# KwonGihyun/TweedieMix

Hardware: AMD Instinct MI355X
Metric: denoise steps/sec @ SDXL 1024^2 K=3 concepts (fusion phase); images/sec at 1/2/4/8 GPUs (higher is better)
Workload: dtype bf16

## Files before the change

include/tmix.h:

```cpp
#ifndef TMIX_H
#define TMIX_H

#include <stdint.h>

#ifdef __cplusplus
extern "C" {
#endif

#define TMIX_VERSION 100

enum { TMIX_OK = 0, TMIX_EINVAL = -1, TMIX_ESHAPE = -2, TMIX_EARCH = -3, TMIX_EALIGN = -4 };
enum { TMIX_F32 = 0, TMIX_F16 = 1, TMIX_BF16 = 2 };

int tmix_version(void);
const char* tmix_last_error_string(void);
int tmix_check_device(void);
void tmix_env_refresh(void);

int tmix_prof_begin(uint64_t* slots, int capacity, int detail);
int tmix_prof_end(void);

enum { TMIX_STEP_FUSION = 0, TMIX_STEP_PLAIN = 1, TMIX_STEP_RESAMPLE = 2 };
int tmix_fused_tweedie_step(const float* x, const void* eps, int eps_dtype, const float* masks,
                            float* out_x, float* out_x0, int K, int channels, int64_t hw, int mode,
// ... 10 lines not shown
int tmix_video_step_prologue(const float* x, float* x_u, int64_t clip_stride_u, float* t_u, float* x_c, int64_t clip_stride_c,
                             float* t_c, const float* params, int videos, int channels, int frames, int64_t hw, int row_channels,
                             void* stream);
int tmix_vpred_step_dev(float* x, const float* v_u, int64_t clip_stride_u, const float* v_c, int64_t clip_stride_c,
                        const float* params, int videos, int channels, int frames, int64_t hw, void* stream);
int tmix_frame_inject(void* x, int dtype, int clips, int frames, int64_t per_frame, int hard, float interp,
                      float one_minus_interp, void* stream);

enum { TMIX_EPI_NONE = 0, TMIX_EPI_GEGLU = 1, TMIX_EPI_F32OUT = 2 ,
       TMIX_EPI_GELU = 3 ,
       TMIX_EPI_QUICKGELU = 4  };
enum { TMIX_TILE_AUTO = 0, TMIX_TILE_128x128_S2 = 1, TMIX_TILE_256x128_S3 = 2, TMIX_TILE_128x128_S4 = 3,
       TMIX_TILE_256x256_S2 = 4, TMIX_TILE_256x128_W4 = 5, TMIX_TILE_256x256_W4 = 6, TMIX_TILE_128x160_S2 = 7,
       TMIX_TILE_128x160_S2_LW = 8, TMIX_TILE_256x128_S3_LW = 9, TMIX_TILE_128x128_S2_LW = 10, TMIX_TILE_256x256_S2_LW = 11,
       TMIX_TILE_128x160_S4 = 12 ,
       TMIX_TILE_64x160_W5 = 13 ,
       TMIX_TILE_256x320_S2 = 14 ,
       TMIX_TILE_32x160_W5 = 15 ,
       TMIX_TILE_256x256_PH = 16 ,
       TMIX_TILE_256x128_PH = 17,
       TMIX_TILE_128x160_S4_K2 = 18 ,
       TMIX_TILE_128x160_S3_LW = 19 ,
       TMIX_TILE_128x160_S4_LW2 = 20 ,
       TMIX_TILE_128x160_S4_LW4 = 21 ,
       TMIX_TILE_256x320_PH = 22 ,
       TMIX_TILE_128x160_W22 = 23 ,
       TMIX_TILE_CONV_HALO = 26 ,
       TMIX_TILE_COUNT = 26 };
typedef struct {
    const void* A;  int64_t lda, strideA;
    const void* W;  int64_t ldw, strideW;
    void*       C;  int64_t ldc, strideC;
    const float* bias;  int64_t strideBias;
    const void* residual; int64_t ldr, strideR;
    const float* rowgroup_bias;
    int32_t rows_per_group;
    void*   Ct; int64_t ldct, strideCt;
    int32_t n_trans_begin;
    int32_t M, N, K, batch;
    int32_t epilogue;
    int32_t tile_cfg;
    float* row_stats_out; int64_t strideStatsOut, ldStatsOut;
    const float* ln_stats; int64_t strideLnStats, ldLnStats;
    const float* ln_colsum; int64_t strideLnColsum;
    float ln_inv_c, ln_eps;
    int32_t ln_parts, reserved0;
    float* col_stats_out;
    int32_t w_period, reserved1;
} tmix_gemm_desc;
int tmix_gemm_bf16(const tmix_gemm_desc* d, void* stream);
int tmix_gemm_resolve_tile(const tmix_gemm_desc* d, int fp8_operands);
int tmix_gemm_f8copy_tile(int tile_cfg);
int tmix_gemm_prefetch_next(const void* next_weights, int64_t bytes, void* stream);
enum { TMIX_F8_A_BLOCK_SCALES = 1, TMIX_F8_GEGLU_OUT = 2, TMIX_F8_COPY_OUT = 4 };
#define TMIX_COLSTATS_ROWS 32
int tmix_gemm_fp8(const tmix_gemm_desc* d, const uint8_t* scale_a, const uint8_t* scale_w, void* stream);
int tmix_gemm_q_cross_attn(const tmix_gemm_desc* d, const void* K, int64_t ldk, int64_t strideK, const void* Vt, int64_t ldvt, int64_t strideVt,
                           void* O, int64_t ldo, int rows_per_image, int Skv, float scale, void* stream);
int tmix_quantize_fp8_rows(const void* X, int64_t ld, void* Q, int64_t ldq, uint8_t* scale_e8m0, int64_t rows, int K, void* stream);
int tmix_gemm_tile_shape(int tile_cfg, int* bm, int* bn);
int tmix_gemm_stats_parts(int N, int tile_cfg);

enum { TMIX_CONV_S1 = 0, TMIX_CONV_S2 = 1, TMIX_CONV_UP2 = 2, TMIX_CONV_T3 = 3, TMIX_CONV_S2A = 4 };
typedef struct {
    const void* X;
    const void* Wt;
    void*       Y;
    const float* bias;
    const float* batch_bias;
    const void* residual;
    int32_t B, H, W, Cin, Cout, mode;
    int32_t tile_cfg;
    int32_t batch_bias_images;
    float* col_stats_out;
    const void* S1; const void* S2;
    int32_t S1_channels, S2_channels;
} tmix_conv_desc;
int tmix_conv3x3_nhwc(const tmix_conv_desc* d, void* stream);
int tmix_conv3x3_nhwc_fp8(const tmix_conv_desc* d, const uint8_t* scale_x, const uint8_t* scale_w, void* stream);
int tmix_conv_resolve_tile(const tmix_conv_desc* d, int fp8_operands);

int tmix_conv_in(const float* x_nchw, const float* w_ohwi, const float* bias, void* y_nhwc,
                 int B, int Cin, int H, int W, int Cout, void* stream);
int tmix_conv_in_pre(const float* x_nchw, const float* w_ohwi, const float* bias, void* y_nhwc,
                     int B, int Cin, int H, int W, int Cout, const float* pre_w, const float* pre_b, void* stream);
int tmix_conv_out(const void* x_nhwc, const void* w_ohwi, const float* bias, float* y_nchw,
                  int B, int Cin, int H, int W, int Cout, void* stream);

int tmix_attn_fwd(const void* Q, int64_t ldq, int64_t strideQ, const void* K, int64_t ldk, int64_t strideK,
                  const void* Vt, int64_t ldvt, int64_t strideVt, void* O, int64_t ldo, int64_t strideO,
                  int B, int H, int Sq, int Skv, float scale, void* stream);
int tmix_attn_fwd_f8(const void* Q, int64_t ldq, int64_t strideQ, const void* K, int64_t ldk, int64_t strideK,
                     const void* Vt, int64_t ldvt, int64_t strideVt, void* O8, int64_t ldo8, void* scales, int64_t ldScale,
                     int B, int H, int Sq, int Skv, float scale, void* stream);
int64_t tmix_attn_split_ws_bytes(int B, int H, int Sq, int Skv);
int tmix_attn_fwd_ws(const void* Q, int64_t ldq, int64_t strideQ, const void* K, int64_t ldk, int64_t strideK,
                     const void* Vt, int64_t ldvt, int64_t strideVt, void* O, int64_t ldo, int64_t strideO,
                     int B, int H, int Sq, int Skv, float scale, void* ws, int64_t ws_bytes, void* stream);
int tmix_attn_fwd_f8_ws(const void* Q, int64_t ldq, int64_t strideQ, const void* K, int64_t ldk, int64_t strideK,
                        const void* Vt, int64_t ldvt, int64_t strideVt, void* O8, int64_t ldo8, void* scales, int64_t ldScale,
                        int B, int H, int Sq, int Skv, float scale, void* ws, int64_t ws_bytes, void* stream);

int64_t tmix_groupnorm_ws_floats(int B, int C, int groups);
int tmix_groupnorm_ws_chunks(int64_t HW);
int tmix_groupnorm_nhwc(const void* X1, int C1, const void* X2, int C2, void* Y, const float* gamma,
                        const float* beta, float* ws, int B, int64_t HW, int groups, float eps, int silu,
                        void* stream);
int tmix_groupnorm_nhwc_launches(int64_t HW, int C, int groups);
int tmix_groupnorm_nhwc_pre(const void* X1, int C1, const void* X2, int C2, void* Y, const float* gamma,
                            const float* beta, float* ws, int B, int64_t HW, int groups, float eps, int silu,
                            const float* cs1, int cs1_channels, const float* cs2, int cs2_channels, void* stream);
int tmix_groupnorm_nhwc_pre_f8(const void* X1, int C1, const void* X2, int C2, void* Y8, void* scales, const float* gamma,
                               const float* beta, float* ws, int B, int64_t HW, int groups, float eps, int silu,
                               const float* cs1, int cs1_channels, const float* cs2, int cs2_channels, void* stream);
int tmix_layernorm(const void* X, void* Y, const float* gamma, const float* beta, int64_t rows, int C,
                   float eps, void* stream);
int tmix_zero(void* ptr, int64_t nbytes, void* stream);
int tmix_concat_channels(const void* X1, int C1, const void* X2, int C2, void* Y, int64_t rows, void* stream);
int tmix_timestep_embedding(const float* values, float* out, int count, int dim, void* stream);
int tmix_softmax_rows(const float* S, int64_t ld_s, void* P, int64_t ld_p, int64_t rows, int cols, float scale, void* stream);
int tmix_softmax_rows_causal(const float* S, int64_t ld_s, void* P, int64_t ld_p, int64_t rows, int cols, float scale,
                             int seq, void* stream);
int tmix_softmax_rows_masked(const float* S, int64_t ld_s, void* P, int64_t ld_p, int64_t rows, int cols, int valid, float scale,
                             void* stream);
int tmix_temporal_attn(const void* QKV, int64_t ld, void* O, int64_t ldo, int clips, int frames, int64_t hw, int heads,
                       float scale, void* stream);
int tmix_lora_down(void* A, int64_t lda, int K, int64_t rows, const void* D, int P, int nsets, const float* dcolsum, const float* dbias,
                   float eps, const int* sets, int64_t rows_per_set, void* stream);
int tmix_affine_clamp(const float* x, float* y, int64_t n, float scale, float shift, float lo, float hi, void* stream);
int tmix_linear_small(const float* in, const void* W, const float* bias, const float* add, float* out,
                      int M, int N, int K, int act_in, int act_out, void* stream);
int tmix_linear_small_sections(const float* in, const void* W, const float* bias, float* out, int M, int N, int K,
                               int act_in, const int* sec_starts, int nsec, void* stream);

int tmix_conv3x3_f32(const float* x_nchw, const float* w_oihw, const float* bias, float* y_nchw, int B, int Cin, int H, int W, int Cout,
                     int stride, int silu, void* stream);
int tmix_adaptive_avgpool_f32(const float* x, float* y, int64_t planes, int H, int W, int OH, int OW, void* stream);
int tmix_linear_f32(const float* in, const float* W, const float* bias, float* out, int M, int N, int K, int act_in, int act_out, void* stream);
int tmix_i2v_temporal_encoder(const float* x, float* y, int clips, int frames, int channels, int64_t hw, const float* ln_gamma, const float* ln_beta,
                              const float* wq, const float* wk, const float* wv, const float* wo, const float* bo,
                              const float* w1, const float* b1, const float* w2, const float* b2, void* stream);

int tmix_xattn_token_maps(const void* Q, int64_t ldq, int64_t strideQ, const void* K, int64_t ldk, int64_t strideK, float* maps,
                          int B, int H, int Sq, int Lk, int row0, int row_step, int n_rows, const int32_t* tokens, int n_tok,
                          int accumulate, float scale, void* stream);

#ifdef __cplusplus
}
#endif
#endif
```

tweediemix_amd/csrc/norm_misc.hip:

```cpp
#include "common.h"

namespace {

typedef __attribute__((ext_vector_type(8))) __bf16 frag_ab;

__device__ __forceinline__ void unpack8(const uint4& v, float (&f)[8]) {
    f[0] = bf2f((bf16_t)(v.x & 0xffff)); f[1] = bf2f((bf16_t)(v.x >> 16));
    f[2] = bf2f((bf16_t)(v.y & 0xffff)); f[3] = bf2f((bf16_t)(v.y >> 16));
    f[4] = bf2f((bf16_t)(v.z & 0xffff)); f[5] = bf2f((bf16_t)(v.z >> 16));
    f[6] = bf2f((bf16_t)(v.w & 0xffff)); f[7] = bf2f((bf16_t)(v.w >> 16));
}
__device__ __forceinline__ uint4 pack8(const float (&f)[8]) {
    uint4 v;
    v.x = pack_bf2(f[0], f[1]); v.y = pack_bf2(f[2], f[3]); v.z = pack_bf2(f[4], f[5]); v.w = pack_bf2(f[6], f[7]);
    return v;
}

constexpr int GN_MAX_C = 4096;

#ifndef GN_T
#define GN_T 128
#endif
#ifndef GN_APPLY_U
#define GN_APPLY_U 2
// ... 61 lines not shown
        float* o = ws + (((int64_t)b * chunks + ch) * groups + tid) * 2;
        o[0] = s; o[1] = q;
    }
}

__global__ void __launch_bounds__(64) gn_finalize_kernel(const float* __restrict__ ws, const float* __restrict__ gamma,
                                                         const float* __restrict__ beta, float2* __restrict__ ss,
                                                         int C, int64_t HW, int groups, int chunks, float eps) {
    const int g = blockIdx.x, b = blockIdx.y, lane = threadIdx.x, cpg = C / groups;
    double s = 0.0, q = 0.0;
    for (int ch = lane; ch < chunks; ch += 64) {
        const float* o = ws + (((int64_t)b * chunks + ch) * groups + g) * 2;
        s += (double)o[0]; q += (double)o[1];
    }
#pragma unroll
    for (int o = 32; o > 0; o >>= 1) { s += __shfl_xor(s, o); q += __shfl_xor(q, o); }
    const double n = (double)HW * cpg;
    const double mean = s / n;
    double var = q / n - mean * mean; if (var < 0.0) var = 0.0;
    const float meanf = (float)mean, rstd = (float)(1.0 / sqrt(var + (double)eps));
    for (int c = g * cpg + lane; c < (g + 1) * cpg; c += 64) {
        const float sc = rstd * gamma[c];
        ss[(int64_t)b * C + c] = make_float2(sc, beta[c] - meanf * sc);
    }
}

constexpr int GN_CS_T = 1024;
__device__ __forceinline__ void gn_cs_walk(const float* __restrict__ base, int Cs, int n, int nblk, int tid, float& s, float& q) {
    if (n <= 0) return;
    const int J = GN_CS_T / n, j = tid / n, c = tid - j * n;
    if (j >= J) return;
    const float* row = base + (int64_t)j * 2 * Cs + c;
    const int64_t step = (int64_t)J * 2 * Cs;
    int blk = j;
    for (; blk + 3 * J < nblk; blk += 4 * J, row += 4 * step) {
        const float a0 = row[0], b0 = row[Cs], a1 = row[step], b1 = row[step + Cs];
        const float a2 = row[2 * step], b2 = row[2 * step + Cs], a3 = row[3 * step], b3 = row[3 * step + Cs];
        s += (a0 + a1) + (a2 + a3); q += (b0 + b1) + (b2 + b3);
    }
    for (; blk < nblk; blk += J, row += step) { s += row[0]; q += row[Cs]; }
}
__global__ void __launch_bounds__(GN_CS_T) gn_finalize_cs_kernel(const float* __restrict__ cs1, int C1, const float* __restrict__ cs2, int C2,
                                                                 const float* __restrict__ gamma, const float* __restrict__ beta,
                                                                 float2* __restrict__ ss, int64_t HW, int groups, float eps,
                                                                 unsigned long long* prof) {
    __shared__ double s_red[2 * GN_CS_T / 64];
    __shared__ float s_ms[2];
    if (prof && threadIdx.x == 0) prof_enter(prof, (blockIdx.x | blockIdx.y) == 0, 0);
    const int C = C1 + C2, cpg = C / groups;
    const int g = blockIdx.x, b = blockIdx.y, tid = threadIdx.x;
    const int nblk = (int)(HW / 32);
    float gm = 0.f, bt = 0.f;
    if (tid < cpg) { gm = gamma[g * cpg + tid]; bt = beta[g * cpg + tid]; }
    const int c_lo = g * cpg, c_hi = c_lo + cpg;
    const int n1 = min(c_hi, C1) - min(c_lo, C1), n2 = cpg - n1;
    float s = 0.f, q = 0.f;
    gn_cs_walk(cs1 + (int64_t)b * nblk * 2 * C1 + c_lo, C1, n1, nblk, tid, s, q);
    if (n2 > 0) gn_cs_walk(cs2 + (int64_t)b * nblk * 2 * C2 + (max(c_lo, C1) - C1), C2, n2, nblk, tid, s, q);
    double sd = (double)s, qd = (double)q;
#pragma unroll
    for (int o = 32; o > 0; o >>= 1) { sd += __shfl_xor(sd, o); qd += __shfl_xor(qd, o); }
    if ((tid & 63) == 0) { s_red[(tid >> 6) * 2] = sd; s_red[(tid >> 6) * 2 + 1] = qd; }
    __syncthreads();
    if (tid == 0) {
        double st = 0.0, qt = 0.0;
#pragma unroll
        for (int w = 0; w < GN_CS_T / 64; ++w) { st += s_red[2 * w]; qt += s_red[2 * w + 1]; }
        const double n = (double)HW * cpg;
        const double mean = st / n;
        double var = qt / n - mean * mean; if (var < 0.0) var = 0.0;
        s_ms[0] = (float)mean; s_ms[1] = (float)(1.0 / sqrt(var + (double)eps));
    }
    __syncthreads();
    if (tid < cpg) {
        const float sc = s_ms[1] * gm;
        ss[(int64_t)b * C + c_lo + tid] = make_float2(sc, bt - s_ms[0] * sc);
    }
}

__device__ __forceinline__ float silu_fast(float x) {
    return x * __builtin_amdgcn_rcpf(1.0f + __builtin_amdgcn_exp2f(-1.4426950408889634f * x));
}

__device__ __forceinline__ float gn_quad_max(float x) {
    float y = __int_as_float(__builtin_amdgcn_update_dpp(0, __float_as_int(x), 0xB1, 0xf, 0xf, false));
    x = fmaxf(x, y);
    y = __int_as_float(__builtin_amdgcn_update_dpp(0, __float_as_int(x), 0x4E, 0xf, 0xf, false));
    return fmaxf(x, y);
}

template <int F8>
__global__ void __launch_bounds__(256) gn_apply_kernel(const bf16_t* __restrict__ X1, int C1, const bf16_t* __restrict__ X2, int C2,
                                                       bf16_t* __restrict__ Y, const float2* __restrict__ ss, int64_t HW, int silu,
                                                       unsigned long long* prof, unsigned char* __restrict__ Y8 = nullptr, unsigned char* __restrict__ S8 = nullptr) {
    __shared__ float2 s_ss[GN_MAX_C];
    const unsigned long long pt0 = (prof && threadIdx.x == 0) ? prof_now() : 0;
    const int C = C1 + C2, nvec = C >> 3;
    const int b = blockIdx.y, tid = threadIdx.x;
    for (int c = tid; c < C; c += 256) s_ss[c] = ss[(int64_t)b * C + c];
    __syncthreads();
    const int64_t total = HW * nvec;
    int64_t per = (total + gridDim.x - 1) / gridDim.x;
    if (F8) per = (per + 3) & ~(int64_t)3;
    const int64_t i0 = (int64_t)blockIdx.x * per;
    int64_t i1 = i0 + per; if (i1 > total) i1 = total;
    int64_t p = i0 / nvec; int v = (int)(i0 - p * nvec) + tid;
    while (v >= nvec) { v -= nvec; ++p; }
    const int step_p = 256 / nvec, step_v = 256 - step_p * nvec;
    constexpr int U = GN_APPLY_U;
    for (int64_t i = i0 + tid; i < i1; i += 256 * U) {
        uint4 raw[U]; int64_t pp[U]; int cc[U];
#pragma unroll
        for (int u = 0; u < U; ++u) {
            pp[u] = p; cc[u] = v * 8;
            if (i + u * 256 < i1) {
                const bf16_t* src = (cc[u] < C1) ? X1 + ((int64_t)b * HW + p) * C1 + cc[u] : X2 + ((int64_t)b * HW + p) * C2 + (cc[u] - C1);
                raw[u] = *(const uint4*)src;
            }
            p += step_p; v += step_v;
            if (v >= nvec) { v -= nvec; ++p; }
        }
#pragma unroll
        for (int u = 0; u < U; ++u) {
            if (i + u * 256 < i1) {
                float f[8]; unpack8(raw[u], f);
#pragma unroll
                for (int j = 0; j < 8; ++j) {
                    const float2 k = s_ss[cc[u] + j];
                    float y = f[j] * k.x + k.y;
                    if (silu) y = silu_fast(y);
                    f[j] = y;
                }
                if constexpr (F8) {
                    const uint4 pk = pack8(f);
                    unpack8(pk, f);
                    float am = 0.f;
#pragma unroll
                    for (int j = 0; j < 8; ++j) am = fmaxf(am, fabsf(f[j]));
                    am = gn_quad_max(am);
                    const int e = e8m0_for_amax(am);
                    const float inv = exp2_neg_int(e);
                    int q0 = __builtin_amdgcn_cvt_pk_fp8_f32(f[0] * inv, f[1] * inv, 0, false); q0 = __builtin_amdgcn_cvt_pk_fp8_f32(f[2] * inv, f[3] * inv, q0, true);
                    int q1 = __builtin_amdgcn_cvt_pk_fp8_f32(f[4] * inv, f[5] * inv, 0, false); q1 = __builtin_amdgcn_cvt_pk_fp8_f32(f[6] * inv, f[7] * inv, q1, true);
                    const int64_t row = (int64_t)b * HW + pp[u];
                    *(uint2*)(Y8 + row * C + cc[u]) = make_uint2((unsigned)q0, (unsigned)q1);
                    if ((tid & 3) == 0) S8[row * (C >> 5) + (cc[u] >> 5)] = (unsigned char)(e + 127);
                } else
                *(uint4*)(Y + ((int64_t)b * HW + pp[u]) * C + cc[u]) = pack8(f);
            }
        }
    }
    if (prof && threadIdx.x == 0) prof_leave(prof, 0, pt0, pt0, pt0);
}

constexpr int GN_SMALL_MAX_CW = 256, GN_SMALL_MAX_ELEMS = 65536;
__global__ void __launch_bounds__(256) gn_small_kernel(const bf16_t* __restrict__ X1, int C1, const bf16_t* __restrict__ X2, int C2, bf16_t* __restrict__ Y,
                                                       const float* __restrict__ gamma, const float* __restrict__ beta, int HW, int groups, int gpw, float eps, int silu,
                                                       unsigned long long* prof) {
    __shared__ float r_s[2048], r_q[2048];
    __shared__ double c_s[GN_SMALL_MAX_CW], c_q[GN_SMALL_MAX_CW];
    __shared__ float g_ms[16];
    __shared__ float2 s_ss[GN_SMALL_MAX_CW];
    const unsigned long long pt0 = (prof && threadIdx.x == 0) ? prof_enter(prof, (blockIdx.x | blockIdx.y) == 0, 0) : 0;
    const int C = C1 + C2, cpg = C / groups, cw = gpw * cpg, nv = cw >> 3, rs = 256 / nv;
    const int b = blockIdx.y, c0 = blockIdx.x * cw, tid = threadIdx.x;
    const int v = tid % nv, slot = tid / nv;
    const bool active = slot < rs;
    const int cg = c0 + v * 8;
    const bf16_t* src; int ld;
    if (cg < C1) { src = X1 + (int64_t)b * HW * C1 + cg; ld = C1; } else { src = X2 + (int64_t)b * HW * C2 + (cg - C1); ld = C2; }
    float s[8], q[8];
#pragma unroll
    for (int j = 0; j < 8; ++j) { s[j] = 0.f; q[j] = 0.f; }
    if (active) {
        int row = slot;
        for (; row + 3 * rs < HW; row += 4 * rs) {
            uint4 raw[4];
#pragma unroll
            for (int u = 0; u < 4; ++u) raw[u] = *(const uint4*)(src + (int64_t)(row + u * rs) * ld);
#pragma unroll
            for (int u = 0; u < 4; ++u) {
                float f[8]; unpack8(raw[u], f);
#pragma unroll
                for (int j = 0; j < 8; ++j) { s[j] += f[j]; q[j] += f[j] * f[j]; }
            }
        }
        for (; row < HW; row += rs) {
            float f[8]; unpack8(*(const uint4*)(src + (int64_t)row * ld), f);
#pragma unroll
            for (int j = 0; j < 8; ++j) { s[j] += f[j]; q[j] += f[j] * f[j]; }
        }
#pragma unroll
        for (int j = 0; j < 8; ++j) { r_s[slot * cw + v * 8 + j] = s[j]; r_q[slot * cw + v * 8 + j] = q[j]; }
    }
    __syncthreads();
    if (tid < cw) {
        double a = 0.0, d = 0.0;
        for (int k = 0; k < rs; ++k) { a += (double)r_s[k * cw + tid]; d += (double)r_q[k * cw + tid]; }
        c_s[tid] = a; c_q[tid] = d;
    }
    __syncthreads();
    if (tid < gpw) {
        double a = 0.0, d = 0.0;
        for (int k = 0; k < cpg; ++k) { a += c_s[tid * cpg + k]; d += c_q[tid * cpg + k]; }
        const double n = (double)HW * cpg, mean = a / n;
        double var = d / n - mean * mean; if (var < 0.0) var = 0.0;
        g_ms[2 * tid] = (float)mean; g_ms[2 * tid + 1] = (float)(1.0 / sqrt(var + (double)eps));
    }
    __syncthreads();
    if (tid < cw) {
        const int g = tid / cpg;
        const float sc = g_ms[2 * g + 1] * gamma[c0 + tid];
        s_ss[tid] = make_float2(sc, beta[c0 + tid] - g_ms[2 * g] * sc);
    }
    __syncthreads();
    if (active) {
        float2 k[8];
#pragma unroll
        for (int j = 0; j < 8; ++j) k[j] = s_ss[v * 8 + j];
        bf16_t* dst = Y + (int64_t)b * HW * C + cg;
        int row = slot;
        for (; row + 3 * rs < HW; row += 4 * rs) {
            uint4 raw[4];
#pragma unroll
            for (int u = 0; u < 4; ++u) raw[u] = *(const uint4*)(src + (int64_t)(row + u * rs) * ld);
#pragma unroll
            for (int u = 0; u < 4; ++u) {
                float f[8]; unpack8(raw[u], f);
#pragma unroll
                for (int j = 0; j < 8; ++j) { float y = f[j] * k[j].x + k[j].y; if (silu) y = silu_fast(y); f[j] = y; }
                *(uint4*)(dst + (int64_t)(row + u * rs) * C) = pack8(f);
            }
        }
        for (; row < HW; row += rs) {
            float f[8]; unpack8(*(const uint4*)(src + (int64_t)row * ld), f);
#pragma unroll
            for (int j = 0; j < 8; ++j) { float y = f[j] * k[j].x + k[j].y; if (silu) y = silu_fast(y); f[j] = y; }
            *(uint4*)(dst + (int64_t)row * C) = pack8(f);
        }
    }
    if (prof && threadIdx.x == 0) prof_leave(prof, 0, pt0, pt0, pt0);
}
static int gn_small_gpw(int64_t HW, int C, int groups) {
    if (tmix_env(TMIX_ENV_GN_NO_SMALL)) return 0;
    const int cpg = C / groups;
    for (int gpw = 1; gpw <= 8; gpw <<= 1) {
        if (groups % gpw || ((gpw * cpg) & 7)) continue;
        const int cw = gpw * cpg;
        if (cw > GN_SMALL_MAX_CW || HW * cw > GN_SMALL_MAX_ELEMS) return 0;
        return gpw;
    }
    return 0;
}

__global__ void __launch_bounds__(256) layernorm_kernel(const bf16_t* __restrict__ X, bf16_t* __restrict__ Y,
                                                        const float* __restrict__ gamma, const float* __restrict__ beta,
                                                        int64_t rows, int C, float eps) {
    const int lane = threadIdx.x & 63;
    const int64_t row = (int64_t)blockIdx.x * 4 + (threadIdx.x >> 6);
    if (row >= rows) return;
    const int nvec = C >> 3;
    float f[4][8];
    float s = 0.f;
#pragma unroll
    for (int i = 0; i < 4; ++i) {
        const int v = i * 64 + lane;
        if (v < nvec) {
            const uint4 raw = *(const uint4*)(X + row * C + v * 8);
            unpack8(raw, f[i]);
#pragma unroll
            for (int j = 0; j < 8; ++j) s += f[i][j];
        }
    }
#pragma unroll
    for (int o = 32; o > 0; o >>= 1) s += __shfl_xor(s, o);
    const float mean = s / (float)C;
    float q = 0.f;
#pragma unroll
    for (int i = 0; i < 4; ++i) {
        const int v = i * 64 + lane;
        if (v < nvec) {
#pragma unroll
            for (int j = 0; j < 8; ++j) { const float d = f[i][j] - mean; q += d * d; }
        }
    }
#pragma unroll
    for (int o = 32; o > 0; o >>= 1) q += __shfl_xor(q, o);
    const float rstd = rsqrtf(q / (float)C + eps);
#pragma unroll
    for (int i = 0; i < 4; ++i) {
        const int v = i * 64 + lane;
        if (v < nvec) {
            const float4 g0 = *(const float4*)(gamma + v * 8), g1 = *(const float4*)(gamma + v * 8 + 4);
            const float4 b0 = *(const float4*)(beta + v * 8), b1 = *(const float4*)(beta + v * 8 + 4);
            const float gg[8] = {g0.x, g0.y, g0.z, g0.w, g1.x, g1.y, g1.z, g1.w};
            const float bb[8] = {b0.x, b0.y, b0.z, b0.w, b1.x, b1.y, b1.z, b1.w};
            float y[8];
#pragma unroll
            for (int j = 0; j < 8; ++j) y[j] = (f[i][j] - mean) * rstd * gg[j] + bb[j];
            *(uint4*)(Y + row * C + v * 8) = pack8(y);
        }
    }
}

__global__ void __launch_bounds__(256) softmax_rows_kernel(const float* __restrict__ S, int64_t ld_s, bf16_t* __restrict__ P,
                                                           int64_t ld_p, int cols, float scale_log2e, int seq, int valid) {
    __shared__ float red[4];
    const float* row = S + (int64_t)blockIdx.x * ld_s;
    bf16_t* out = P + (int64_t)blockIdx.x * ld_p;
    const int tid = threadIdx.x, lane = tid & 63, w = tid >> 6;
    const int lim = seq > 0 ? (int)(blockIdx.x % (unsigned)seq) + 1 : valid;
    auto load = [&](int c) {
        float4 v = *(const float4*)(row + c);
        if (c + 0 >= lim) v.x = -INFINITY;
        if (c + 1 >= lim) v.y = -INFINITY;
        if (c + 2 >= lim) v.z = -INFINITY;
        if (c + 3 >= lim) v.w = -INFINITY;
        return v;
    };
    float mx = -INFINITY;
    for (int c = tid * 4; c < cols; c += 1024) {
        const float4 v = load(c);
        mx = fmaxf(fmaxf(mx, fmaxf(v.x, v.y)), fmaxf(v.z, v.w));
    }
#pragma unroll
    for (int o = 32; o > 0; o >>= 1) mx = fmaxf(mx, __shfl_xor(mx, o));
    if (lane == 0) red[w] = mx;
    __syncthreads();
    mx = fmaxf(fmaxf(red[0], red[1]), fmaxf(red[2], red[3])) * scale_log2e;
    __syncthreads();
    float sum = 0.f;
    for (int c = tid * 4; c < cols; c += 1024) {
        const float4 v = load(c);
        sum += exp2f(v.x * scale_log2e - mx) + exp2f(v.y * scale_log2e - mx) + exp2f(v.z * scale_log2e - mx) + exp2f(v.w * scale_log2e - mx);
    }
// ... 63 lines not shown
                float xf[8] = {x0.x, x0.y, x0.z, x0.w, x1.x, x1.y, x1.z, x1.w};
                if (act_in) {
#pragma unroll
                    for (int j = 0; j < 8; ++j) xf[j] = silu_f(xf[j]);
                }
#pragma unroll
                for (int j = 0; j < 8; ++j) acc[m] += xf[j] * wf[j];
            }
        }
    }
#pragma unroll
    for (int m = 0; m < MAXM; ++m) {
#pragma unroll
        for (int o = 32; o > 0; o >>= 1) acc[m] += __shfl_xor(acc[m], o);
    }
    if (lane == 0) {
        int64_t base = 0; int ldn = N, col = n;
        if (secs) {
            int sidx = 0;
            while (sidx + 1 < nsec && secs[sidx + 1] <= n) ++sidx;
            base = (int64_t)secs[sidx] * Mtot; ldn = secs[sidx + 1] - secs[sidx]; col = n - secs[sidx];
        }
        for (int m = 0; m < M; ++m) {
            float y = acc[m] + (bias ? bias[n] : 0.f) + (add ? add[(int64_t)m * N + n] : 0.f);
            if (act_out) y = silu_f(y);
            out[base + (int64_t)(secs ? mrow0 + m : m) * ldn + col] = y;
        }
    }
}

struct PreMap { float w[16]; float b[4]; int on; };

template <int CIN>
__global__ void __launch_bounds__(256) conv_in_kernel(const float* __restrict__ x, const float* __restrict__ w,
                                                      const float* __restrict__ bias, bf16_t* __restrict__ y,
                                                      int B, int H, int W, int Cout, const PreMap pm) {
    extern __shared__ __attribute__((aligned(16))) float s_w[];
    constexpr int KK = 9 * CIN;
    const int tid = threadIdx.x, lane = tid & 63;
    const int q = __builtin_amdgcn_readfirstlane(tid >> 6);
    for (int i = tid; i < Cout * KK / 4; i += 256) ((float4*)s_w)[i] = ((const float4*)w)[i];
    __syncthreads();
    const int64_t npix = (int64_t)B * H * W;
    for (int64_t tile = blockIdx.x; tile * 64 < npix; tile += gridDim.x) {
    int64_t pix = tile * 64 + lane;
    const bool live = pix < npix;
    if (!live) pix = npix - 1;
    const int b = (int)(pix / ((int64_t)H * W)); const int rem = (int)(pix - (int64_t)b * H * W);
    const int oy = rem / W, ox = rem - oy * W;
    float patch[KK];
#pragma unroll
    for (int ky = 0; ky < 3; ++ky)
#pragma unroll
        for (int kx = 0; kx < 3; ++kx) {
            const int iy = oy + ky - 1, ix = ox + kx - 1;
            const bool ok = iy >= 0 && iy < H && ix >= 0 && ix < W;
            float v[CIN];
#pragma unroll
            for (int ci = 0; ci < CIN; ++ci) v[ci] = ok ? x[(((int64_t)b * CIN + ci) * H + iy) * W + ix] : 0.f;
            if (pm.on && CIN == 4) {
                float u[4];
#pragma unroll
                for (int co = 0; co < 4; ++co)
                    u[co] = ok ? pm.b[co] + pm.w[co * 4 + 0] * v[0] + pm.w[co * 4 + 1] * v[1] + pm.w[co * 4 + 2] * v[2] + pm.w[co * 4 + 3] * v[3] : 0.f;
#pragma unroll
                for (int co = 0; co < 4; ++co) v[co] = u[co];
            }
#pragma unroll
            for (int ci = 0; ci < CIN; ++ci) patch[(ky * 3 + kx) * CIN + ci] = v[ci];
        }
    const int cpq = Cout / 4;
    for (int c0 = q * cpq; c0 < (q + 1) * cpq; c0 += 8) {
        float o[8];
#pragma unroll 2
        for (int j = 0; j < 8; ++j) {
            const float* wr = s_w + (c0 + j) * KK;
            float a = bias ? bias[c0 + j] : 0.f;
#pragma unroll
            for (int k = 0; k < KK; ++k) a += patch[k] * wr[k];
            o[j] = a;
        }
        if (live) *(uint4*)(y + pix * Cout + c0) = pack8(o);
    }
    }
}

__global__ void __launch_bounds__(256) conv_out_kernel(const bf16_t* __restrict__ x, const bf16_t* __restrict__ w,
                                                       const float* __restrict__ bias, float* __restrict__ y,
                                                       int B, int H, int W, int Cin, int Cout) {
    const int lane = threadIdx.x & 63, fr = lane & 15, fg = lane >> 4;
    const int64_t npix = (int64_t)B * H * W;
    const int64_t pbase = ((int64_t)blockIdx.x * 4 + (threadIdx.x >> 6)) * 16;
    if (pbase >= npix) return;
    int64_t pix = pbase + fr; if (pix > npix - 1) pix = npix - 1;
    const int b = (int)(pix / ((int64_t)H * W)); const int rem = (int)(pix - (int64_t)b * H * W);
    const int oy = rem / W, ox = rem - oy * W;
    const int co = fr < Cout ? fr : Cout - 1;
    const bf16_t* wrow = w + (int64_t)co * 9 * Cin;
    f32x4 acc = {0.f, 0.f, 0.f, 0.f};
    const frag_ab zero = {0, 0, 0, 0, 0, 0, 0, 0};
    for (int tap = 0; tap < 9; ++tap) {
        const int ky = tap / 3, kx = tap - ky * 3;
        const int iy = oy + ky - 1, ix = ox + kx - 1;
        const bool ok = iy >= 0 && iy < H && ix >= 0 && ix < W;
        const bf16_t* src = x + (((int64_t)b * H + (ok ? iy : 0)) * W + (ok ? ix : 0)) * Cin;
        for (int c = 0; c < Cin; c += 32) {
            frag_ab a = *(const frag_ab*)(src + c + fg * 8);
            if (!ok) a = zero;
            const frag_ab wf = *(const frag_ab*)(wrow + tap * Cin + c + fg * 8);
            acc = __builtin_amdgcn_mfma_f32_16x16x32_bf16(a, wf, acc, 0, 0, 0);
        }
    }
    if (fr < Cout) {
        const float bv = bias ? bias[fr] : 0.f;
#pragma unroll
        for (int r = 0; r < 4; ++r) {
            const int64_t pp = pbase + fg * 4 + r;
            if (pp < npix) {
                const int bb = (int)(pp / ((int64_t)H * W)); const int64_t rr = pp - (int64_t)bb * H * W;
                y[((int64_t)bb * Cout + fr) * H * W + rr] = acc[r] + bv;
            }
        }
    }
}

}

extern "C" int tmix_groupnorm_ws_chunks(int64_t HW) { return gn_chunks(HW); }
extern "C" int64_t tmix_groupnorm_ws_floats(int B, int C, int groups) { return (int64_t)B * GN_T * groups * 2 + (int64_t)B * C * 2; }

extern "C" int tmix_groupnorm_nhwc_launches(int64_t HW, int C, int groups) {
    if (HW <= 0 || C <= 0 || groups <= 0 || (C % groups)) return 0;
    return gn_small_gpw(HW, C, groups) ? 1 : 3;
}

extern "C" int tmix_groupnorm_nhwc(const void* X1, int C1, const void* X2, int C2, void* Y, const float* gamma,
                                   const float* beta, float* ws, int B, int64_t HW, int groups, float eps, int silu,
                                   void* stream) {
    if (!X1 || !Y || !gamma || !beta || !ws) TMIX_FAIL(TMIX_EINVAL, "groupnorm: null pointer");
    if (C2 > 0 && !X2) TMIX_FAIL(TMIX_EINVAL, "groupnorm: C2 > 0 but X2 is null");
    const int C = C1 + C2;
    if (B <= 0 || HW <= 0 || C <= 0) TMIX_FAIL(TMIX_ESHAPE, "groupnorm: empty problem");
    if ((C1 % 8) || (C2 % 8) || C > GN_MAX_C || groups <= 0 || groups > 64 || (C % groups)) TMIX_FAIL(TMIX_ESHAPE, "groupnorm: C1=%d C2=%d groups=%d unsupported", C1, C2, groups);
    if (!aligned16(X1) || (X2 && !aligned16(X2)) || !aligned16(Y)) TMIX_FAIL(TMIX_EALIGN, "groupnorm: pointers must be 16-byte aligned");
    const int chunks = gn_chunks(HW);
    hipStream_t st = (hipStream_t)stream;
    unsigned long long* prof = tmix_prof_take();
    if (const int gpw = gn_small_gpw(HW, C, groups)) {
        gn_small_kernel<<<dim3(groups / gpw, B), 256, 0, st>>>((const bf16_t*)X1, C1, (const bf16_t*)X2, C2, (bf16_t*)Y, gamma, beta, (int)HW, groups, gpw, eps, silu, prof);
        TMIX_LAUNCH_CHECK();
        return TMIX_OK;
    }
    gn_stats_kernel<<<dim3(chunks, B), 256, 0, st>>>((const bf16_t*)X1, C1, (const bf16_t*)X2, C2, ws, HW, groups, chunks, prof);
    TMIX_LAUNCH_CHECK();
    float2* ss = (float2*)(ws + (int64_t)B * GN_T * groups * 2);
    gn_finalize_kernel<<<dim3(groups, B), 64, 0, st>>>(ws, gamma, beta, ss, C, HW, groups, chunks, eps);
    TMIX_LAUNCH_CHECK();
    int64_t nb = (HW * (C / 8) + GN_APPLY_ITEMS - 1) / GN_APPLY_ITEMS; if (nb < 1) nb = 1; if (nb > GN_APPLY_MAXB) nb = GN_APPLY_MAXB;
    gn_apply_kernel<0><<<dim3((unsigned)nb, B), 256, 0, st>>>((const bf16_t*)X1, C1, (const bf16_t*)X2, C2, (bf16_t*)Y, ss, HW, silu, prof);
    TMIX_LAUNCH_CHECK();
    return TMIX_OK;
}

static int gn_pre_entry(const void* X1, int C1, const void* X2, int C2, void* Y, void* S8, const float* gamma,
                        const float* beta, float* ws, int B, int64_t HW, int groups, float eps, int silu,
                        const float* cs1, int cs1_channels, const float* cs2, int cs2_channels, void* stream) {
    if (!X1 || !Y || !gamma || !beta || !ws || !cs1) TMIX_FAIL(TMIX_EINVAL, "groupnorm_pre: null pointer");
    if (S8 && ((C1 + C2) % 32)) TMIX_FAIL(TMIX_ESHAPE, "groupnorm_pre_f8: C must be a multiple of 32 (MX blocks)");
    if (C2 > 0 && !X2) TMIX_FAIL(TMIX_EINVAL, "groupnorm_pre: C2 > 0 but X2 is null");
    const int C = C1 + C2;
    if (cs1_channels <= 0 || cs2_channels < 0 || cs1_channels + cs2_channels != C || (cs2_channels > 0 && !cs2))
        TMIX_FAIL(TMIX_EINVAL, "groupnorm_pre: the partials cover %d + %d channels, the tensor has %d", cs1_channels, cs2_channels, C);
    if (B <= 0 || HW <= 0 || C <= 0) TMIX_FAIL(TMIX_ESHAPE, "groupnorm_pre: empty problem");
    if ((C1 % 8) || (C2 % 8) || C > GN_MAX_C || groups <= 0 || groups > 64 || (C % groups) || C / groups > 256) TMIX_FAIL(TMIX_ESHAPE, "groupnorm_pre: C1=%d C2=%d groups=%d unsupported", C1, C2, groups);
    if (HW % TMIX_COLSTATS_ROWS) TMIX_FAIL(TMIX_ESHAPE, "groupnorm_pre: HW=%lld must be a multiple of %d (the producers' partials cover 32-row blocks)", (long long)HW, TMIX_COLSTATS_ROWS);
    if (!aligned16(X1) || (X2 && !aligned16(X2)) || !aligned16(Y)) TMIX_FAIL(TMIX_EALIGN, "groupnorm_pre: pointers must be 16-byte aligned");
    hipStream_t st = (hipStream_t)stream;
    unsigned long long* prof = tmix_prof_take();
    float2* ss = (float2*)(ws + (int64_t)B * GN_T * groups * 2);
    gn_finalize_cs_kernel<<<dim3(groups, B), GN_CS_T, 0, st>>>(cs1, cs1_channels, cs2, cs2_channels, gamma, beta, ss, HW, groups, eps, prof);
    TMIX_LAUNCH_CHECK();
    int64_t nb = (HW * (C / 8) + GN_APPLY_ITEMS - 1) / GN_APPLY_ITEMS; if (nb < 1) nb = 1; if (nb > GN_APPLY_MAXB) nb = GN_APPLY_MAXB;
    if (S8) gn_apply_kernel<1><<<dim3((unsigned)nb, B), 256, 0, st>>>((const bf16_t*)X1, C1, (const bf16_t*)X2, C2, nullptr, ss, HW, silu, prof, (unsigned char*)Y, (unsigned char*)S8);
    else gn_apply_kernel<0><<<dim3((unsigned)nb, B), 256, 0, st>>>((const bf16_t*)X1, C1, (const bf16_t*)X2, C2, (bf16_t*)Y, ss, HW, silu, prof);
    TMIX_LAUNCH_CHECK();
    return TMIX_OK;
}

extern "C" int tmix_groupnorm_nhwc_pre(const void* X1, int C1, const void* X2, int C2, void* Y, const float* gamma,
                                       const float* beta, float* ws, int B, int64_t HW, int groups, float eps, int silu,
                                       const float* cs1, int cs1_channels, const float* cs2, int cs2_channels, void* stream) {
    return gn_pre_entry(X1, C1, X2, C2, Y, nullptr, gamma, beta, ws, B, HW, groups, eps, silu, cs1, cs1_channels, cs2, cs2_channels, stream);
}

extern "C" int tmix_groupnorm_nhwc_pre_f8(const void* X1, int C1, const void* X2, int C2, void* Y8, void* scales, const float* gamma,
                                          const float* beta, float* ws, int B, int64_t HW, int groups, float eps, int silu,
                                          const float* cs1, int cs1_channels, const float* cs2, int cs2_channels, void* stream) {
    if (!scales) TMIX_FAIL(TMIX_EINVAL, "groupnorm_pre_f8: null scale array");
    return gn_pre_entry(X1, C1, X2, C2, Y8, scales, gamma, beta, ws, B, HW, groups, eps, silu, cs1, cs1_channels, cs2, cs2_channels, stream);
}

extern "C" int tmix_layernorm(const void* X, void* Y, const float* gamma, const float* beta, int64_t rows, int C,
                              float eps, void* stream) {
    if (!X || !Y || !gamma || !beta) TMIX_FAIL(TMIX_EINVAL, "layernorm: null pointer");
    if (rows <= 0 || C <= 0) TMIX_FAIL(TMIX_ESHAPE, "layernorm: empty problem");
    if ((C % 8) || C > 2048) TMIX_FAIL(TMIX_ESHAPE, "layernorm: C=%d must be a multiple of 8 and <= 2048", C);
    if (!aligned16(X) || !aligned16(Y) || !aligned16(gamma) || !aligned16(beta)) TMIX_FAIL(TMIX_EALIGN, "layernorm: pointers must be 16-byte aligned");
    layernorm_kernel<<<(unsigned)((rows + 3) / 4), 256, 0, (hipStream_t)stream>>>((const bf16_t*)X, (bf16_t*)Y, gamma, beta, rows, C, eps);
    TMIX_LAUNCH_CHECK();
    return TMIX_OK;
}

__global__ void __launch_bounds__(256) quantize_fp8_rows_kernel(const bf16_t* __restrict__ X, int64_t ld, unsigned char* __restrict__ Q, int64_t ldq,
                                                                unsigned char* __restrict__ scale, int64_t rows, int K) {
    const int lane = threadIdx.x & 63;
    const int64_t r = (int64_t)blockIdx.x * 4 + (threadIdx.x >> 6);
    if (r >= rows) return;
    constexpr int MAXV = 16;
    const int nv = K >> 3;
    uint4 v[MAXV];
    float amax = 0.f;
#pragma unroll
    for (int u = 0; u < MAXV; ++u) {
        const int c = u * 64 + lane;
        if (c < nv) {
            v[u] = *(const uint4*)(X + r * ld + (int64_t)c * 8);
            const unsigned w[4] = {v[u].x, v[u].y, v[u].z, v[u].w};
#pragma unroll
            for (int k = 0; k < 4; ++k) amax = fmaxf(amax, fmaxf(fabsf(__uint_as_float(w[k] << 16)), fabsf(__uint_as_float(w[k] & 0xffff0000u))));
        }
    }
#pragma unroll
    for (int off = 32; off >= 1; off >>= 1) amax = fmaxf(amax, __shfl_xor(amax, off));
    const int e = e8m0_for_amax(amax);
    const float inv = exp2_neg_int(e);
    if (lane == 0) scale[r] = (unsigned char)(e + 127);
#pragma unroll
    for (int u = 0; u < MAXV; ++u) {
        const int c = u * 64 + lane;
        if (c < nv) {
            const unsigned w[4] = {v[u].x, v[u].y, v[u].z, v[u].w};
            unsigned o[2];
#pragma unroll
            for (int h = 0; h < 2; ++h) {
                const float f0 = __uint_as_float(w[2 * h] << 16) * inv, f1 = __uint_as_float(w[2 * h] & 0xffff0000u) * inv;
                const float f2 = __uint_as_float(w[2 * h + 1] << 16) * inv, f3 = __uint_as_float(w[2 * h + 1] & 0xffff0000u) * inv;
                int pk = __builtin_amdgcn_cvt_pk_fp8_f32(f0, f1, 0, false);
                pk = __builtin_amdgcn_cvt_pk_fp8_f32(f2, f3, pk, true);
                o[h] = (unsigned)pk;
            }
            *(uint2*)(Q + r * ldq + (int64_t)c * 8) = make_uint2(o[0], o[1]);
        }
    }
}

extern "C" int tmix_quantize_fp8_rows(const void* X, int64_t ld, void* Q, int64_t ldq, uint8_t* scale_e8m0, int64_t rows, int K, void* stream) {
    if (!X || !Q || !scale_e8m0) TMIX_FAIL(TMIX_EINVAL, "quantize_fp8_rows: null pointer");
    if (rows <= 0 || K <= 0 || (K % 8) || K > 8192) TMIX_FAIL(TMIX_ESHAPE, "quantize_fp8_rows: rows=%lld K=%d (K %% 8 == 0, K <= 8192)", (long long)rows, K);
    if (!aligned16(X) || (ld % 8) || (((uintptr_t)Q) & 7) || (ldq % 8)) TMIX_FAIL(TMIX_EALIGN, "quantize_fp8_rows: X rows must be 16-byte, Q rows 8-byte aligned");
    quantize_fp8_rows_kernel<<<(unsigned)((rows + 3) / 4), 256, 0, (hipStream_t)stream>>>((const bf16_t*)X, ld, (unsigned char*)Q, ldq, scale_e8m0, rows, K);
    TMIX_LAUNCH_CHECK();
    return TMIX_OK;
}

extern "C" int tmix_zero(void* ptr, int64_t nbytes, void* stream) {
    if (!ptr || nbytes <= 0) TMIX_FAIL(TMIX_EINVAL, "zero: null pointer / empty range");
    hipError_t e = hipMemsetAsync(ptr, 0, (size_t)nbytes, (hipStream_t)stream);
    if (e != hipSuccess) TMIX_FAIL((int)e, "hipMemsetAsync: %s", hipGetErrorString(e));
    return TMIX_OK;
}

extern "C" int tmix_concat_channels(const void* X1, int C1, const void* X2, int C2, void* Y, int64_t rows, void* stream) {
    if (!X1 || !X2 || !Y) TMIX_FAIL(TMIX_EINVAL, "concat: null pointer");
    if (rows <= 0 || C1 <= 0 || C2 <= 0 || (C1 % 8) || (C2 % 8)) TMIX_FAIL(TMIX_ESHAPE, "concat: rows=%lld C1=%d C2=%d unsupported", (long long)rows, C1, C2);
    if (!aligned16(X1) || !aligned16(X2) || !aligned16(Y)) TMIX_FAIL(TMIX_EALIGN, "concat: pointers must be 16-byte aligned");
    int64_t nb = (rows * ((C1 + C2) / 8) + 255) / 256; if (nb > 4096) nb = 4096;
    concat_kernel<<<(unsigned)nb, 256, 0, (hipStream_t)stream>>>((const uint4*)X1, C1 / 8, (const uint4*)X2, C2 / 8, (uint4*)Y, rows);
    TMIX_LAUNCH_CHECK();
    return TMIX_OK;
}

namespace {
// ... 200 lines not shown
extern "C" int tmix_timestep_embedding(const float* values, float* out, int count, int dim, void* stream) {
    if (!values || !out) TMIX_FAIL(TMIX_EINVAL, "timestep_embedding: null pointer");
    if (count <= 0 || dim <= 0 || (dim & 1)) TMIX_FAIL(TMIX_ESHAPE, "timestep_embedding: count=%d dim=%d", count, dim);
    const int n = count * (dim / 2);
    timestep_embedding_kernel<<<(n + 255) / 256, 256, 0, (hipStream_t)stream>>>(values, out, count, dim);
    TMIX_LAUNCH_CHECK();
    return TMIX_OK;
}

static int linear_small_launch(const float* in, const void* W, const float* bias, const float* add, float* out, int M, int N, int K,
                               int act_in, int act_out, const int* secs, int nsec, hipStream_t st) {
    for (int m0 = 0; m0 < M; m0 += 16) {
        const int m = M - m0 < 16 ? M - m0 : 16;
        const float* in_c = in + (int64_t)m0 * K;
        const float* add_c = add ? add + (int64_t)m0 * N : nullptr;
        float* out_c = secs ? out : out + (int64_t)m0 * N;
        if (m <= 4) linear_small_kernel<4><<<(N + 3) / 4, 256, 0, st>>>(in_c, (const bf16_t*)W, bias, add_c, out_c, m, N, K, act_in, act_out, secs, nsec, M, m0);
        else        linear_small_kernel<16><<<(N + 3) / 4, 256, 0, st>>>(in_c, (const bf16_t*)W, bias, add_c, out_c, m, N, K, act_in, act_out, secs, nsec, M, m0);
        TMIX_LAUNCH_CHECK();
    }
    return TMIX_OK;
}

extern "C" int tmix_linear_small(const float* in, const void* W, const float* bias, const float* add, float* out,
                                 int M, int N, int K, int act_in, int act_out, void* stream) {
    if (!in || !W || !out) TMIX_FAIL(TMIX_EINVAL, "linear_small: null pointer");
    if (M <= 0 || M > 256 || N <= 0 || K <= 0 || (K % 8)) TMIX_FAIL(TMIX_ESHAPE, "linear_small: M=%d (1..256) N=%d K=%d (K %% 8 == 0)", M, N, K);
    if (!aligned16(in) || !aligned16(W)) TMIX_FAIL(TMIX_EALIGN, "linear_small: in/W must be 16-byte aligned");
    return linear_small_launch(in, W, bias, add, out, M, N, K, act_in, act_out, nullptr, 0, (hipStream_t)stream);
}

extern "C" int tmix_linear_small_sections(const float* in, const void* W, const float* bias, float* out, int M, int N, int K,
                                          int act_in, const int* sec_starts, int nsec, void* stream) {
    if (!in || !W || !out || !sec_starts) TMIX_FAIL(TMIX_EINVAL, "linear_small_sections: null pointer");
    if (M <= 0 || M > 256 || N <= 0 || K <= 0 || (K % 8) || nsec < 1) TMIX_FAIL(TMIX_ESHAPE, "linear_small_sections: M=%d (1..256) N=%d K=%d (K %% 8 == 0) nsec=%d", M, N, K, nsec);
    if (!aligned16(in) || !aligned16(W)) TMIX_FAIL(TMIX_EALIGN, "linear_small_sections: in/W must be 16-byte aligned");
    return linear_small_launch(in, W, bias, nullptr, out, M, N, K, act_in, 0, sec_starts, nsec, (hipStream_t)stream);
}

extern "C" int tmix_conv_in(const float* x_nchw, const float* w_ohwi, const float* bias, void* y_nhwc,
                            int B, int Cin, int H, int W, int Cout, void* stream) {
    return tmix_conv_in_pre(x_nchw, w_ohwi, bias, y_nhwc, B, Cin, H, W, Cout, nullptr, nullptr, stream);
}

extern "C" int tmix_conv_in_pre(const float* x_nchw, const float* w_ohwi, const float* bias, void* y_nhwc,
                                int B, int Cin, int H, int W, int Cout, const float* pre_w, const float* pre_b, void* stream) {
    if (!x_nchw || !w_ohwi || !y_nhwc) TMIX_FAIL(TMIX_EINVAL, "conv_in: null pointer");
    if (B <= 0 || H <= 0 || W <= 0 || Cout <= 0) TMIX_FAIL(TMIX_ESHAPE, "conv_in: bad shape");
    if (!aligned16(y_nhwc)) TMIX_FAIL(TMIX_EALIGN, "conv_in: output must be 16-byte aligned");
    if (Cout % 32) TMIX_FAIL(TMIX_ESHAPE, "conv_in: Cout=%d must be a multiple of 32", Cout);
    if (Cin != 3 && Cin != 4 && Cin != 8) TMIX_FAIL(TMIX_ESHAPE, "conv_in: Cin=%d (3: RGB image, 4: image latent, 8: video latent + image-latent features)", Cin);
    if (Cin != 4 && pre_w) TMIX_FAIL(TMIX_EINVAL, "conv_in: the latent pre-map is defined for 4 channels");
    if ((Cout * 9 * Cin) % 4) TMIX_FAIL(TMIX_ESHAPE, "conv_in: Cout*9*Cin must be a multiple of 4");
    if (!aligned16(w_ohwi)) TMIX_FAIL(TMIX_EALIGN, "conv_in: weights must be 16-byte aligned");
    const int64_t npix = (int64_t)B * H * W;
    const int64_t ntiles = (npix + 63) / 64;
    const int smem = Cout * 9 * Cin * 4;
    const int per_cu = smem > 80 * 1024 ? 1 : (smem > 52 * 1024 ? 2 : 3);
    const unsigned nb = (unsigned)(ntiles < 256 * per_cu ? ntiles : 256 * per_cu);
    if (smem > 150 * 1024) TMIX_FAIL(TMIX_ESHAPE, "conv_in: Cout=%d too large for the LDS weight stage", Cout);
    static int attr_smem[3] = {0, 0, 0};
    const int slot = Cin == 8 ? 2 : (Cin == 4 ? 1 : 0);
    if (smem > 64 * 1024 && smem > attr_smem[slot]) {
        hipError_t e = Cin == 8 ? hipFuncSetAttribute((const void*)conv_in_kernel<8>, hipFuncAttributeMaxDynamicSharedMemorySize, smem)
                     : Cin == 4 ? hipFuncSetAttribute((const void*)conv_in_kernel<4>, hipFuncAttributeMaxDynamicSharedMemorySize, smem)
                                : hipFuncSetAttribute((const void*)conv_in_kernel<3>, hipFuncAttributeMaxDynamicSharedMemorySize, smem);
        if (e != hipSuccess) TMIX_FAIL((int)e, "hipFuncSetAttribute: %s", hipGetErrorString(e));
        attr_smem[slot] = smem;
    }
    PreMap pm = {};
    if (pre_w) {
        pm.on = 1;
        for (int i = 0; i < 16; ++i) pm.w[i] = pre_w[i];
        for (int i = 0; i < 4; ++i) pm.b[i] = pre_b ? pre_b[i] : 0.f;
    }
    hipStream_t st = (hipStream_t)stream;
    if (Cin == 8) conv_in_kernel<8><<<nb, 256, smem, st>>>(x_nchw, w_ohwi, bias, (bf16_t*)y_nhwc, B, H, W, Cout, pm);
    else if (Cin == 3) conv_in_kernel<3><<<nb, 256, smem, st>>>(x_nchw, w_ohwi, bias, (bf16_t*)y_nhwc, B, H, W, Cout, pm);
    else          conv_in_kernel<4><<<nb, 256, smem, st>>>(x_nchw, w_ohwi, bias, (bf16_t*)y_nhwc, B, H, W, Cout, pm);
    TMIX_LAUNCH_CHECK();
    return TMIX_OK;
}

extern "C" int tmix_conv_out(const void* x_nhwc, const void* w_ohwi, const float* bias, float* y_nchw,
                             int B, int Cin, int H, int W, int Cout, void* stream) {
    if (!x_nhwc || !w_ohwi || !y_nchw) TMIX_FAIL(TMIX_EINVAL, "conv_out: null pointer");
    if (B <= 0 || H <= 0 || W <= 0 || Cout <= 0 || Cout > 16 || (Cin % 32)) TMIX_FAIL(TMIX_ESHAPE, "conv_out: Cin=%d (%%32) Cout=%d (<=16)", Cin, Cout);
    if (!aligned16(x_nhwc) || !aligned16(w_ohwi)) TMIX_FAIL(TMIX_EALIGN, "conv_out: pointers must be 16-byte aligned");
    const int64_t npix = (int64_t)B * H * W;
    const unsigned nb = (unsigned)((npix + 63) / 64);
    conv_out_kernel<<<nb, 256, 0, (hipStream_t)stream>>>((const bf16_t*)x_nhwc, (const bf16_t*)w_ohwi, bias, y_nchw, B, H, W, Cin, Cout);
    TMIX_LAUNCH_CHECK();
    return TMIX_OK;
}
```

tweediemix_amd/lib.py:

```python
from __future__ import annotations

import ctypes as C
import os

_HERE = os.path.dirname(os.path.abspath(__file__))
LIB_PATH = os.path.join(_HERE, "lib", "libtmix_hip.so")
LIB_PATH = os.environ.get("TMIX_LIB", LIB_PATH)

OK, EINVAL, ESHAPE, EARCH, EALIGN = 0, -1, -2, -3, -4
F32, F16, BF16 = 0, 1, 2
STEP_FUSION, STEP_PLAIN, STEP_RESAMPLE = 0, 1, 2
EPI_NONE, EPI_GEGLU, EPI_F32OUT, EPI_GELU, EPI_QUICKGELU = 0, 1, 2, 3, 4
CONV_S1, CONV_S2, CONV_UP2, CONV_T3, CONV_S2A = 0, 1, 2, 3, 4
F8_A_BLOCK_SCALES, F8_GEGLU_OUT, F8_COPY_OUT = 1, 2, 4
TILE_AUTO, TILE_COUNT = 0, 26
TILE_CANDIDATES = (1, 2, 3, 4, 5, 7, 12, 13, 14, 15, 16, 17, 18, 19, 20, 21, 22)
TILE_EXCLUSIVE = (13, 14, 15, 22, 24)
TILE_CONV_HALO = 26

i32, i64, f32, vp = C.c_int32, C.c_int64, C.c_float, C.c_void_p


class GemmDesc(C.Structure):
    _fields_ = [("A", vp), ("lda", i64), ("strideA", i64),
                ("W", vp), ("ldw", i64), ("strideW", i64),
                ("C", vp), ("ldc", i64), ("strideC", i64),
                ("bias", vp), ("strideBias", i64),
                ("residual", vp), ("ldr", i64), ("strideR", i64),
                ("rowgroup_bias", vp), ("rows_per_group", i32),
                ("Ct", vp), ("ldct", i64), ("strideCt", i64),
                ("n_trans_begin", i32),
                ("M", i32), ("N", i32), ("K", i32), ("batch", i32),
                ("epilogue", i32), ("tile_cfg", i32),
                ("row_stats_out", vp), ("strideStatsOut", i64), ("ldStatsOut", i64),
                ("ln_stats", vp), ("strideLnStats", i64), ("ldLnStats", i64),
                ("ln_colsum", vp), ("strideLnColsum", i64), ("ln_inv_c", f32), ("ln_eps", f32),
                ("ln_parts", C.c_int32), ("reserved0", C.c_int32),
                ("col_stats_out", vp), ("w_period", C.c_int32), ("reserved1", C.c_int32)]


class ConvDesc(C.Structure):
    _fields_ = [("X", vp), ("Wt", vp), ("Y", vp), ("bias", vp), ("batch_bias", vp), ("residual", vp),
                ("B", i32), ("H", i32), ("W", i32), ("Cin", i32), ("Cout", i32), ("mode", i32), ("tile_cfg", i32),
                ("batch_bias_images", i32), ("col_stats_out", vp), ("S1", vp), ("S2", vp), ("S1_channels", i32), ("S2_channels", i32)]


SIGNATURES = {
    "tmix_version": (C.c_int, []),
    "tmix_last_error_string": (C.c_char_p, []),
    "tmix_check_device": (C.c_int, []),
    "tmix_env_refresh": (None, []),
    "tmix_prof_begin": (C.c_int, [vp, C.c_int, C.c_int]),
    "tmix_prof_end": (C.c_int, []),
    "tmix_fused_tweedie_step": (C.c_int, [vp, vp, C.c_int, vp, vp, vp, C.c_int, C.c_int, i64, C.c_int,
                                          f32, f32, f32, f32, f32, C.c_int, vp]),
    "tmix_fused_tweedie_step_dev": (C.c_int, [vp, vp, C.c_int, vp, i64, vp, vp, C.c_int, C.c_int, i64, C.c_int, C.c_int,
                                              C.c_int, vp, vp]),
    "tmix_step_prologue": (C.c_int, [vp, vp, vp, vp, C.c_int, C.c_int, i64, vp]),
    "tmix_gemm_bf16": (C.c_int, [C.POINTER(GemmDesc), vp]),
    "tmix_gemm_prefetch_next": (C.c_int, [vp, i64, vp]),
    "tmix_gemm_fp8": (C.c_int, [C.POINTER(GemmDesc), vp, vp, vp]),
    "tmix_gemm_q_cross_attn": (C.c_int, [C.POINTER(GemmDesc), vp, i64, i64, vp, i64, i64, vp, i64, C.c_int, C.c_int, f32, vp]),
    "tmix_quantize_fp8_rows": (C.c_int, [vp, i64, vp, i64, vp, i64, C.c_int, vp]),
    "tmix_conv3x3_nhwc": (C.c_int, [C.POINTER(ConvDesc), vp]),
    "tmix_conv3x3_nhwc_fp8": (C.c_int, [C.POINTER(ConvDesc), vp, vp, vp]),
    "tmix_conv_in": (C.c_int, [vp, vp, vp, vp, C.c_int, C.c_int, C.c_int, C.c_int, C.c_int, vp]),
    "tmix_conv_in_pre": (C.c_int, [vp, vp, vp, vp, C.c_int, C.c_int, C.c_int, C.c_int, C.c_int, vp, vp, vp]),
    "tmix_softmax_rows": (C.c_int, [vp, i64, vp, i64, i64, C.c_int, f32, vp]),
    "tmix_softmax_rows_causal": (C.c_int, [vp, i64, vp, i64, i64, C.c_int, f32, C.c_int, vp]),
    "tmix_softmax_rows_masked": (C.c_int, [vp, i64, vp, i64, i64, C.c_int, C.c_int, f32, vp]),
    "tmix_affine_clamp": (C.c_int, [vp, vp, i64, f32, f32, f32, f32, vp]),
    "tmix_conv_out": (C.c_int, [vp, vp, vp, vp, C.c_int, C.c_int, C.c_int, C.c_int, C.c_int, vp]),
    "tmix_attn_fwd": (C.c_int, [vp, i64, i64, vp, i64, i64, vp, i64, i64, vp, i64, i64,
                                C.c_int, C.c_int, C.c_int, C.c_int, f32, vp]),
    "tmix_attn_fwd_f8": (C.c_int, [vp, i64, i64, vp, i64, i64, vp, i64, i64, vp, i64, vp, i64,
                                   C.c_int, C.c_int, C.c_int, C.c_int, f32, vp]),
    "tmix_attn_split_ws_bytes": (i64, [C.c_int, C.c_int, C.c_int, C.c_int]),
    "tmix_attn_fwd_ws": (C.c_int, [vp, i64, i64, vp, i64, i64, vp, i64, i64, vp, i64, i64,
                                   C.c_int, C.c_int, C.c_int, C.c_int, f32, vp, i64, vp]),
    "tmix_attn_fwd_f8_ws": (C.c_int, [vp, i64, i64, vp, i64, i64, vp, i64, i64, vp, i64, vp, i64,
                                      C.c_int, C.c_int, C.c_int, C.c_int, f32, vp, i64, vp]),
    "tmix_groupnorm_nhwc_launches": (C.c_int, [i64, C.c_int, C.c_int]),
    "tmix_groupnorm_ws_chunks": (C.c_int, [i64]),
    "tmix_groupnorm_ws_floats": (i64, [C.c_int, C.c_int, C.c_int]),
    "tmix_groupnorm_nhwc": (C.c_int, [vp, C.c_int, vp, C.c_int, vp, vp, vp, vp, C.c_int, i64, C.c_int, f32,
                                      C.c_int, vp]),
    "tmix_groupnorm_nhwc_pre": (C.c_int, [vp, C.c_int, vp, C.c_int, vp, vp, vp, vp, C.c_int, i64, C.c_int, f32,
                                          C.c_int, vp, C.c_int, vp, C.c_int, vp]),
    "tmix_groupnorm_nhwc_pre_f8": (C.c_int, [vp, C.c_int, vp, C.c_int, vp, vp, vp, vp, vp, C.c_int, i64, C.c_int, f32,
                                             C.c_int, vp, C.c_int, vp, C.c_int, vp]),
    "tmix_layernorm": (C.c_int, [vp, vp, vp, vp, i64, C.c_int, f32, vp]),
    "tmix_zero": (C.c_int, [vp, i64, vp]),
    "tmix_temporal_attn": (C.c_int, [vp, i64, vp, i64, C.c_int, C.c_int, i64, C.c_int, f32, vp]),
    "tmix_vpred_step": (C.c_int, [vp, vp, vp, C.c_int, i64, f32, f32, f32, f32, f32, vp]),
    "tmix_frame_inject": (C.c_int, [vp, C.c_int, C.c_int, C.c_int, i64, C.c_int, f32, f32, vp]),
    "tmix_video_step_prologue": (C.c_int, [vp, vp, i64, vp, vp, i64, vp, vp, C.c_int, C.c_int, C.c_int, i64, C.c_int, vp]),
    "tmix_vpred_step_dev": (C.c_int, [vp, vp, i64, vp, i64, vp, C.c_int, C.c_int, C.c_int, i64, vp]),
    "tmix_gemm_tile_shape": (C.c_int, [C.c_int, C.POINTER(C.c_int), C.POINTER(C.c_int)]),
    "tmix_gemm_stats_parts": (C.c_int, [C.c_int, C.c_int]),
    "tmix_gemm_resolve_tile": (C.c_int, [C.POINTER(GemmDesc), C.c_int]),
    "tmix_conv_resolve_tile": (C.c_int, [C.POINTER(ConvDesc), C.c_int]),
    "tmix_gemm_f8copy_tile": (C.c_int, [C.c_int]),
    "tmix_concat_channels": (C.c_int, [vp, C.c_int, vp, C.c_int, vp, i64, vp]),
    "tmix_lora_down": (C.c_int, [vp, i64, C.c_int, i64, vp, C.c_int, C.c_int, vp, vp, f32, vp, i64, vp]),
    "tmix_timestep_embedding": (C.c_int, [vp, vp, C.c_int, C.c_int, vp]),
    "tmix_linear_small": (C.c_int, [vp, vp, vp, vp, vp, C.c_int, C.c_int, C.c_int, C.c_int, C.c_int, vp]),
    "tmix_linear_small_sections": (C.c_int, [vp, vp, vp, vp, C.c_int, C.c_int, C.c_int, C.c_int, vp, C.c_int, vp]),
    "tmix_conv3x3_f32": (C.c_int, [vp, vp, vp, vp] + [C.c_int] * 7 + [vp]),
    "tmix_adaptive_avgpool_f32": (C.c_int, [vp, vp, C.c_int64, C.c_int, C.c_int, C.c_int, C.c_int, vp]),
    "tmix_linear_f32": (C.c_int, [vp, vp, vp, vp, C.c_int, C.c_int, C.c_int, C.c_int, C.c_int, vp]),
    "tmix_i2v_temporal_encoder": (C.c_int, [vp, vp, C.c_int, C.c_int, C.c_int, C.c_int64] + [vp] * 11 + [vp]),
    "tmix_xattn_token_maps": (C.c_int, [vp, i64, i64, vp, i64, i64, vp, C.c_int, C.c_int, C.c_int, C.c_int, C.c_int, C.c_int, C.c_int,
                                        C.POINTER(C.c_int32), C.c_int, C.c_int, f32, vp]),
}

_lib = None


class TmixError(RuntimeError):
    pass


def load() -> C.CDLL:
    global _lib
    if _lib is not None:
        return _lib
    import torch
    if not os.path.exists(LIB_PATH):
        raise ImportError(f"{LIB_PATH} not found: build it first (python -c 'import __graft_entry__ as g; g.build()' "
                          f"or make -C tweediemix_amd/csrc). There is no CPU fallback.")
    lib = C.CDLL(LIB_PATH)
    for name, (res, args) in SIGNATURES.items():
        fn = getattr(lib, name)
        fn.restype = res
        fn.argtypes = args
    if lib.tmix_version() != 100:
        raise ImportError(f"libtmix_hip.so ABI version {lib.tmix_version()} != 100")
    _lib = lib
    return lib


def check(rc: int, what: str = "") -> None:
    if rc != 0:
        msg = load().tmix_last_error_string().decode("utf-8", "replace")
        raise TmixError(f"{what} failed with code {rc}: {msg}")
```

tweediemix_amd/ops.py:

```python
from __future__ import annotations

import ctypes as C

import numpy as np
import torch

from . import lib as L

BF16 = torch.bfloat16


def _stream() -> int:
    return torch.cuda.current_stream().cuda_stream


def _p(t):
    return None if t is None else t.data_ptr()


def _need_cuda(*ts):
    for t in ts:
        if t is not None and not t.is_cuda:
            raise L.TmixError("tweediemix_amd ops need device tensors (no CPU fallback exists)")

# ... 232 lines not shown
    if f8_copy is not None:
        f8_copy.attach(d)
    L.check(lib.tmix_gemm_fp8(C.byref(d), sa.data_ptr(), sw.data_ptr(), _stream()), "tmix_gemm_fp8")
    return out if out is not None else kw.get("out_f32")


def make_conv_desc(x, w, out, bias=None, batch_bias=None, residual=None, mode=L.CONV_S1, tile_cfg=0, bias_images=1, col_stats_out=None,
                   shortcut=None, _fp8=False):
    B, H, W, Cin = x.shape
    Cout = w.shape[0]
    dt = torch.uint8 if _fp8 else BF16
    assert x.dtype == dt and w.dtype == dt and x.is_contiguous() and w.is_contiguous() and out.is_contiguous()
    if shortcut is not None:
        s1, s2 = shortcut
        c1, c2 = s1.shape[-1], (0 if s2 is None else s2.shape[-1])
        assert mode == L.CONV_S1 and tuple(w.shape) == (Cout, 9 * Cin + c1 + c2) and residual is None
        assert s1.dtype == BF16 and s1.is_contiguous() and s1.numel() == B * H * W * c1 and (s2 is None or (s2.dtype == BF16 and s2.is_contiguous() and s2.numel() == B * H * W * c2))
    else:
        assert tuple(w.shape) == ((Cout, 3, Cin) if mode == L.CONV_T3 else (Cout, 3, 3, Cin))
    d = L.ConvDesc()
    d.X, d.Wt, d.Y = x.data_ptr(), w.data_ptr(), out.data_ptr()
    d.bias, d.batch_bias, d.residual = _p(bias), _p(batch_bias), _p(residual)
    d.B, d.H, d.W, d.Cin, d.Cout, d.mode = B, H, W, Cin, Cout, mode
    d.tile_cfg = tile_cfg
    d.batch_bias_images = bias_images
    if col_stats_out is not None:
        cs = col_stats_out
        assert cs.dtype == torch.float32 and cs.is_contiguous() and tuple(cs.shape) == (out.numel() // Cout // COLSTATS_ROWS, 2, Cout)
        d.col_stats_out = cs.data_ptr()
    if shortcut is not None:
        d.S1, d.S1_channels = s1.data_ptr(), c1
        if s2 is not None:
            d.S2, d.S2_channels = s2.data_ptr(), c2
    return d


def shortcut_weight(w_conv, w_sc):
    Cout = w_conv.shape[0]
    return torch.cat([w_conv.reshape(Cout, -1), w_sc.reshape(Cout, -1)], dim=1).contiguous()


def conv_out_hw(H, W, mode):
    return (H // 2, W // 2) if mode in (L.CONV_S2, L.CONV_S2A) else ((2 * H, 2 * W) if mode == L.CONV_UP2 else (H, W))


def conv3x3_fp8(x8, sx, w8, sw, bias=None, batch_bias=None, residual=None, mode=L.CONV_S1, out=None, tile_cfg=12, col_stats_out=None, bias_images=1):
    _need_cuda(x8, w8, sx, sw)
    lib = L.load()
    B, H, W, Cin = x8.shape
    Ho, Wo = conv_out_hw(H, W, mode)
    if out is None:
        out = torch.empty(B, Ho, Wo, w8.shape[0], device=x8.device, dtype=BF16)
    assert x8.dtype == torch.uint8 and w8.dtype == torch.uint8 and sx.dtype == torch.uint8 and sw.dtype == torch.uint8
    assert x8.is_contiguous() and w8.is_contiguous() and sx.is_contiguous() and sw.is_contiguous() and sx.numel() == B * H * W * Cin // 32 and sw.numel() == w8.shape[0]
    d = make_conv_desc(x8, w8, out, bias, batch_bias, residual, mode, tile_cfg, bias_images=bias_images, col_stats_out=col_stats_out, _fp8=True)
    L.check(lib.tmix_conv3x3_nhwc_fp8(C.byref(d), sx.data_ptr(), sw.data_ptr(), _stream()), "tmix_conv3x3_nhwc_fp8")
    return out


def conv3x3(x, w, bias=None, batch_bias=None, residual=None, mode=L.CONV_S1, out=None, tile_cfg=0, col_stats_out=None, shortcut=None):
    _need_cuda(x, w)
    lib = L.load()
    B, H, W, _ = x.shape
    Ho, Wo = conv_out_hw(H, W, mode)
    if out is None:
        out = torch.empty(B, Ho, Wo, w.shape[0], device=x.device, dtype=BF16)
    d = make_conv_desc(x, w, out, bias, batch_bias, residual, mode, tile_cfg, col_stats_out=col_stats_out, shortcut=shortcut)
    L.check(lib.tmix_conv3x3_nhwc(C.byref(d), _stream()), "tmix_conv3x3_nhwc")
    return out


def conv_in(x_nchw, w_ohwi, bias, out=None):
    _need_cuda(x_nchw, w_ohwi)
    lib = L.load()
    B, Cin, H, W = x_nchw.shape
    Cout = w_ohwi.shape[0]
    assert x_nchw.dtype == torch.float32 and w_ohwi.dtype == torch.float32 and x_nchw.is_contiguous() and w_ohwi.is_contiguous()
    if out is None:
        out = torch.empty(B, H, W, Cout, device=x_nchw.device, dtype=BF16)
    L.check(lib.tmix_conv_in(_p(x_nchw), _p(w_ohwi), _p(bias), _p(out), B, Cin, H, W, Cout, _stream()), "tmix_conv_in")
    return out


def conv_out(x_nhwc, w_ohwi, bias, out=None):
    _need_cuda(x_nhwc, w_ohwi)
    lib = L.load()
    B, H, W, Cin = x_nhwc.shape
    Cout = w_ohwi.shape[0]
    assert x_nhwc.dtype == BF16 and w_ohwi.dtype == BF16 and x_nhwc.is_contiguous() and w_ohwi.is_contiguous()
    if out is None:
        out = torch.empty(B, Cout, H, W, device=x_nhwc.device, dtype=torch.float32)
    L.check(lib.tmix_conv_out(_p(x_nhwc), _p(w_ohwi), _p(bias), _p(out), B, Cin, H, W, Cout, _stream()), "tmix_conv_out")
    return out


def attention_split_ws(B, H, Sq, Skv, device):
    n = L.load().tmix_attn_split_ws_bytes(B, H, Sq, Skv)
    return torch.zeros(n, device=device, dtype=torch.uint8) if n > 0 else None


def attention(q, k, vt, H, Skv, scale, out=None, f8_out=None, ws=None):
    _need_cuda(q, k, vt)
    lib = L.load()
    B, Sq = q.shape[0], q.shape[1]
    assert q.dtype == BF16 and k.dtype == BF16 and vt.dtype == BF16
    assert q.stride(2) == 1 and k.stride(2) == 1 and vt.stride(2) == 1
    wsa = (ws.data_ptr(), ws.numel()) if ws is not None else (None, 0)
    if f8_out is not None:
        assert f8_out.rows == B * Sq and f8_out.N == H * 64
        L.check(lib.tmix_attn_fwd_f8_ws(_p(q), q.stride(1), q.stride(0), _p(k), k.stride(1), k.stride(0), _p(vt), vt.stride(1), vt.stride(0),
                                        f8_out.q.data_ptr(), f8_out.N, f8_out.scales.data_ptr(), f8_out.rows,
                                        B, H, Sq, Skv, float(scale), *wsa, _stream()), "tmix_attn_fwd_f8_ws")
        return f8_out
    if out is None:
        out = torch.empty(B, Sq, H * 64, device=q.device, dtype=BF16)
    L.check(lib.tmix_attn_fwd_ws(_p(q), q.stride(1), q.stride(0), _p(k), k.stride(1), k.stride(0),
                                 _p(vt), vt.stride(1), vt.stride(0), _p(out), out.stride(1), out.stride(0),
                                 B, H, Sq, Skv, float(scale), *wsa, _stream()), "tmix_attn_fwd_ws")
    return out


def token_array(tokens):
    tokens = [int(t) for t in tokens]
    return (C.c_int32 * max(1, len(tokens)))(*tokens)


def xattn_token_maps(q, k, tokens, H, Lk=None, rows=(0, 1, None), scale=None, out=None, accumulate=False):
    _need_cuda(q, k)
    assert q.dtype == BF16 and k.dtype == BF16 and q.stride(2) == 1 and k.stride(2) == 1
    B, Sq = q.shape[0], q.shape[1]
    Lk = k.shape[1] if Lk is None else Lk
    row0, step, n = rows
    n = len(range(row0, B, step)) if n is None else n
    if out is None:
        out = torch.zeros(n, len(tokens), Sq, device=q.device, dtype=torch.float32)
    assert out.dtype == torch.float32 and out.is_contiguous() and tuple(out.shape) == (n, len(tokens), Sq)
    scale = 64 ** -0.5 if scale is None else scale
    L.check(L.load().tmix_xattn_token_maps(_p(q), q.stride(1), q.stride(0), _p(k), k.stride(1), k.stride(0), _p(out), B, H, Sq, Lk,
                                           row0, step, n, token_array(tokens), len(tokens), int(bool(accumulate)), float(scale),
                                           _stream()), "tmix_xattn_token_maps")
    return out


def groupnorm_ws(B, C, groups, device):
    return torch.empty(L.load().tmix_groupnorm_ws_floats(B, C, groups), device=device, dtype=torch.float32)


def groupnorm(x1, gamma, beta, groups=32, eps=1e-5, silu=False, x2=None, out=None, ws=None, colstats=None, f8_out=None):
    _need_cuda(x1, gamma, beta)
    lib = L.load()
    B, HW, C1 = x1.shape[0], x1.numel() // (x1.shape[0] * x1.shape[-1]), x1.shape[-1]
    C2 = 0 if x2 is None else x2.shape[-1]
    assert x1.is_contiguous() and (x2 is None or x2.is_contiguous()) and gamma.dtype == torch.float32
    assert f8_out is None or colstats is not None, "the e4m3 output exists for the producer-statistics form (tmix_groupnorm_nhwc_pre_f8)"
    if out is None and f8_out is None:
        out = torch.empty(*x1.shape[:-1], C1 + C2, device=x1.device, dtype=BF16)
    if ws is None:
        ws = groupnorm_ws(B, C1 + C2, groups, x1.device)
    if colstats is not None:
        cs1, cs2 = colstats
        ca, cb = cs1.shape[-1], (0 if cs2 is None else cs2.shape[-1])
        assert cs1.is_contiguous() and cs1.shape[1] == 2 and (cs2 is None or (cs2.is_contiguous() and cs2.shape[:2] == cs1.shape[:2]))
        if HW % COLSTATS_ROWS == 0:
            assert cs1.shape[0] == B * HW // COLSTATS_ROWS
        if f8_out is not None:
            y8, s8 = f8_out
            assert y8.dtype == torch.uint8 and s8.dtype == torch.uint8 and y8.is_contiguous() and s8.is_contiguous()
            assert y8.numel() == B * HW * (C1 + C2) and s8.numel() == B * HW * (C1 + C2) // 32
            L.check(lib.tmix_groupnorm_nhwc_pre_f8(_p(x1), C1, _p(x2), C2, _p(y8), _p(s8), _p(gamma), _p(beta), _p(ws), B, HW, groups,
                                                   float(eps), int(bool(silu)), _p(cs1), ca, _p(cs2), cb, _stream()), "tmix_groupnorm_nhwc_pre_f8")
            return f8_out
        L.check(lib.tmix_groupnorm_nhwc_pre(_p(x1), C1, _p(x2), C2, _p(out), _p(gamma), _p(beta), _p(ws), B, HW, groups,
                                            float(eps), int(bool(silu)), _p(cs1), ca, _p(cs2), cb, _stream()), "tmix_groupnorm_nhwc_pre")
        return out
    L.check(lib.tmix_groupnorm_nhwc(_p(x1), C1, _p(x2), C2, _p(out), _p(gamma), _p(beta), _p(ws), B, HW, groups,
                                    float(eps), int(bool(silu)), _stream()), "tmix_groupnorm_nhwc")
    return out


def layernorm(x, gamma, beta, eps=1e-5, out=None):
    _need_cuda(x, gamma, beta)
    lib = L.load()
    Cc = x.shape[-1]
    rows = x.numel() // Cc
    assert x.is_contiguous() and x.dtype == BF16 and gamma.dtype == torch.float32
    if out is None:
        out = torch.empty_like(x)
    L.check(lib.tmix_layernorm(_p(x), _p(out), _p(gamma), _p(beta), rows, Cc, float(eps), _stream()), "tmix_layernorm")
    return out


def concat_channels(x1, x2, out=None):
    _need_cuda(x1, x2)
    lib = L.load()
    C1, C2 = x1.shape[-1], x2.shape[-1]
    rows = x1.numel() // C1
    assert x1.is_contiguous() and x2.is_contiguous() and x1.dtype == BF16 and x2.dtype == BF16
    if out is None:
        out = torch.empty(*x1.shape[:-1], C1 + C2, device=x1.device, dtype=BF16)
    L.check(lib.tmix_concat_channels(_p(x1), C1, _p(x2), C2, _p(out), rows, _stream()), "tmix_concat_channels")
    return out


def timestep_embedding(values, dim, out=None):
    _need_cuda(values)
    lib = L.load()
    assert values.dtype == torch.float32 and values.is_contiguous()
    n = values.numel()
    if out is None:
        out = torch.empty(n, dim, device=values.device, dtype=torch.float32)
    L.check(lib.tmix_timestep_embedding(_p(values), _p(out), n, dim, _stream()), "tmix_timestep_embedding")
    return out


def linear_small_sections(x, w, bias, sec_starts, act_in=False, out=None):
    _need_cuda(x, w, sec_starts)
    lib = L.load()
    M, K = x.shape
    N = w.shape[0]
    assert x.dtype == torch.float32 and x.is_contiguous() and w.dtype == BF16 and w.is_contiguous() and w.shape[1] == K
    assert sec_starts.dtype == torch.int32 and sec_starts.is_contiguous()
    if out is None:
        out = torch.empty(M * N, device=x.device, dtype=torch.float32)
    L.check(lib.tmix_linear_small_sections(_p(x), _p(w), _p(bias), _p(out), M, N, K, int(bool(act_in)), _p(sec_starts),
                                           sec_starts.numel() - 1, _stream()), "tmix_linear_small_sections")
    return out


def linear_small(x, w, bias=None, add=None, act_in=False, act_out=False, out=None):
    _need_cuda(x, w)
    lib = L.load()
    M, K = x.shape
    N = w.shape[0]
    assert x.dtype == torch.float32 and x.is_contiguous() and w.dtype == BF16 and w.is_contiguous() and w.shape[1] == K
    if out is None:
        out = torch.empty(M, N, device=x.device, dtype=torch.float32)
    L.check(lib.tmix_linear_small(_p(x), _p(w), _p(bias), _p(add), _p(out), M, N, K, int(bool(act_in)),
                                  int(bool(act_out)), _stream()), "tmix_linear_small")
    return out


def _f32c(*ts):
    for t in ts:
        assert t is None or (t.dtype == torch.float32 and t.is_contiguous()), "fp32 contiguous tensors"


def conv3x3_f32(x, w, bias=None, stride=1, silu=False):
    _need_cuda(x, w)
    _f32c(x, w, bias)
    B, Ci, H, W_ = x.shape
    Co = w.shape[0]
    assert tuple(w.shape) == (Co, Ci, 3, 3)
    y = torch.empty(B, Co, (H - 1) // stride + 1, (W_ - 1) // stride + 1, device=x.device, dtype=torch.float32)
    L.check(L.load().tmix_conv3x3_f32(_p(x), _p(w), _p(bias), _p(y), B, Ci, H, W_, Co, int(stride), int(bool(silu)), _stream()), "tmix_conv3x3_f32")
    return y


def adaptive_avgpool_f32(x, oh, ow):
    _need_cuda(x)
    _f32c(x)
# ... 131 lines not shown
```

tweediemix_amd/sampler.py:

```python
from __future__ import annotations

from types import SimpleNamespace

import torch

from . import lib as L
from . import ops
from .schedule import Schedule
from .unet import KVCache, PlanGroup, TokenMapSpec, UNetPlan, UNetWeights

F32 = torch.float32


def seed_everything(seed: int):
    import random

    import numpy as np
    torch.manual_seed(seed)
    if torch.cuda.is_available():
        torch.cuda.manual_seed(seed)
    random.seed(seed)
    np.random.seed(seed)


# ... 20 lines not shown
        self.concept_num = int(concept_num)
        self.lora = bool(lora)
        self.strict_reference = strict_reference
        self.use_graphs = use_graphs
        self.n_seeds = int(n_seeds)
        self.n_streams = int(n_streams)
        self.vae = vae
        self.vae_scaling_factor = 0.13025
        self._vae_plans = {}
        self.min_rows_per_stream = 2
        self.text_embeds = text_embeds
        self.text_embeds_single = text_embeds_single
        self.mask_provider = mask_provider
        self.attention_masks = None
        self.attention_maps = None
        self.mask_images = None
        if attention_masks is not None:
            am = dict(attention_masks)
            toks = [[int(p) for p in c] for c in am["tokens"]]
            if len(toks) != self.concept_num - 1 or any(not c for c in toks):
                raise ValueError(f"attention_masks: {len(toks)} token lists for {self.concept_num - 1} foreground concepts")
            flat = [p for c in toks for p in c]
            if len(flat) > 8:
                raise ValueError(f"attention_masks: {len(flat)} token positions, at most 8 in all")
            if int(config.jumping_steps) < 1:
                raise ValueError("attention_masks needs the look-ahead (jumping_steps >= 1): its calls are where the maps come from")
            self.attention_masks = dict(tokens=toks, flat=flat, threshold=float(am.get("threshold", 0.5)),
                                        levels=am.get("levels"), level_weights=am.get("level_weights"))
        self._mask_buf = None
        self.scheduler = Schedule(config.n_timesteps)
        self.skip = self.scheduler.skip
        self.final_alpha_cumprod = self.scheduler.final_alpha_cumprod
        self.h, self.w = config.resolution_h // 8, config.resolution_w // 8
        self.add_time_ids = torch.tensor([[config.resolution_h, config.resolution_w, config.crops_coords_top_left_h,
                                           config.crops_coords_top_left_w, config.resolution_h, config.resolution_w]],
                                         dtype=F32)
        self.plans = {}
        self.graphs = {}
        self.unet_calls = []
        self.preview_x0 = None
        S = self.n_seeds
        self.x_state = torch.zeros(S, 4, self.h, self.w, device=self.device, dtype=F32)
        self.x0_state = torch.zeros_like(self.x_state)
        self._x_backup = torch.zeros_like(self.x_state)
        self.step_params = torch.zeros(8, device=self.device, dtype=F32)
        self._hp = torch.zeros(64, 8, dtype=F32)
        if self.device.type == "cuda":
            self._hp = self._hp.pin_memory()
        self._hp_ev = [None] * self._hp.shape[0]
        self._hp_i = 0
        self._mask_buf = None

    def alpha(self, t):
        return self.scheduler.alpha(int(t))

    def _routes(self, B):
        return B == 4 if self.strict_reference else B == self.concept_num + 1

    def _build_plan(self, kind):
        K = self.concept_num
        te, tp = self.text_embeds
        if kind in ("fusion", "fusion_base"):
            ehs = torch.cat([te[0:1], te[2:2 + K]])
            pooled = torch.cat([tp[0:1], tp[2:2 + K]])
            routed = kind == "fusion" and self._routes(K + 1) and self.W.kind != "none"
            wsel = list(range(K + 1)) if routed else [0] * (K + 1)
        elif kind == "start":
            ts_, tps = self.text_embeds_single
            ehs = torch.cat([te[0:1], te[1:2], ts_[1:K]])
            pooled = torch.cat([tp[0:1], tp[1:2], tps[1:K]])
            routed, wsel = False, [0] * (K + 1)
        elif kind in ("plain", "probe"):
            ehs, pooled, routed, wsel = te[0:2], tp[0:2], False, [0, 0]
        else:
            raise ValueError(kind)
        S = self.n_seeds
        if S > 1:
            ehs, pooled, wsel = ehs.repeat(S, 1, 1), pooled.repeat(S, 1), list(wsel) * S
        B = ehs.shape[0]
        if kind == "probe":
            am = self.attention_masks
            spec = TokenMapSpec(tuple(am["flat"]), row0=1, row_step=2, n_rows=S, levels=am["levels"])
            return UNetPlan(self.W, B, self.h, self.w, KVCache(self.W, ehs, wsel), pooled, self.add_time_ids.repeat(B, 1),
                            fp8=self.fp8, token_maps=spec)
        if self.n_streams > 1 and B % self.n_streams == 0 and B // self.n_streams >= self.min_rows_per_stream:
            return PlanGroup(self.W, self.h, self.w, ehs, wsel, pooled, self.add_time_ids.repeat(B, 1), routed,
                             self.n_streams, fp8=self.fp8)
        kv = KVCache(self.W, ehs, wsel)
        return UNetPlan(self.W, B, self.h, self.w, kv, pooled, self.add_time_ids.repeat(B, 1), routed=routed,
                        row_sets=wsel if routed else None, fp8=self.fp8)

    def plan(self, kind):
        if kind not in self.plans:
            self.plans[kind] = self._build_plan(kind)
        return self.plans[kind]

    def _unet(self, kind, x, t):
        p = self.plan(kind)
        S = self.n_seeds
        self.unet_calls.append((kind, p.B // S, int(t)))
        p.latent.view(S, p.B // S, *p.latent.shape[1:]).copy_(x.unsqueeze(1))
        p.t_dev.fill_(float(t))
        p.run()
        return p.eps

    def _set_masks(self, masks):
        masks = masks.to(self.device, F32).contiguous()
        assert masks.dim() in (4, 5) and tuple(masks.shape[-4:]) == (self.concept_num, 1, self.h, self.w), tuple(masks.shape)
        if self._mask_buf is None or self._mask_buf.shape != masks.shape:
            assert not any(k[1] == L.STEP_FUSION for k in self.graphs), "mask shape changed after the fusion step was captured"
            self._mask_buf = torch.empty_like(masks)
        self._mask_buf.copy_(masks)

    @property
    def masks(self):
        return self._mask_buf

    @masks.setter
    def masks(self, m):
        if m is None:
            self._mask_buf = None
        else:
            self._set_masks(m)

    def _enqueue_step(self, kind, mode):
        p = self.plan(kind)
        S = self.n_seeds
        rows = p.B // S
        n = 4 * self.h * self.w
        lib = L.load()
        st = torch.cuda.current_stream().cuda_stream
        L.check(lib.tmix_step_prologue(self.x_state.data_ptr(), p.latent.data_ptr(), p.t_dev.data_ptr(),
                                       self.step_params.data_ptr(), S, rows, n, st), "tmix_step_prologue")
        p.run()
        m = self._mask_buf if mode == L.STEP_FUSION else None
        mss = 0 if (m is None or m.dim() == 4) else self.concept_num * self.h * self.w
        L.check(lib.tmix_fused_tweedie_step_dev(self.x_state.data_ptr(), p.eps.data_ptr(), L.F32, None if m is None else m.data_ptr(),
                                                mss, self.x_state.data_ptr(), self.x0_state.data_ptr(), self.concept_num, 4,
                                                self.h * self.w, mode, rows, S, self.step_params.data_ptr(), st),
                "tmix_fused_tweedie_step_dev")

    def _run_step(self, kind, mode, t, at, at_next, is_last=False):
        if "_unet" not in vars(self):
            self.unet_calls.append((kind, self.plan(kind).B // self.n_seeds, int(t)))
        sa, s1, san, s1n = ops.step_coeffs(at, at_next)
        i = self._hp_i
        self._hp_i = (i + 1) % self._hp.shape[0]
        if self._hp_ev[i] is not None:
            self._hp_ev[i].synchronize()
        hp = self._hp[i]
        hp[0], hp[1], hp[2], hp[3], hp[4] = float(t), sa, s1, san, s1n
        hp[5], hp[6] = (1.0 if is_last else 0.0), float(self.config.guidance_scale)
        self.step_params.copy_(hp, non_blocking=True)
        if self.device.type == "cuda":
            self._hp_ev[i] = torch.cuda.Event()
            self._hp_ev[i].record()
        if mode == L.STEP_FUSION:
            assert self._mask_buf is not None, "fusion step before the masks were acquired"
        if "_unet" in vars(self):
            eps = self._unet(kind, self.x_state, t).contiguous()
            S = self.n_seeds
            m = self._mask_buf if mode == L.STEP_FUSION else None
            mss = 0 if (m is None or m.dim() == 4) else self.concept_num * self.h * self.w
            L.check(L.load().tmix_fused_tweedie_step_dev(
                self.x_state.data_ptr(), eps.data_ptr(), ops._EPS_DT[eps.dtype], None if m is None else m.data_ptr(), mss,
                self.x_state.data_ptr(), self.x0_state.data_ptr(), self.concept_num, 4, self.h * self.w, mode, eps.shape[0] // S, S,
                self.step_params.data_ptr(), torch.cuda.current_stream().cuda_stream), "tmix_fused_tweedie_step_dev")
            return
        if not self.use_graphs:
            self._enqueue_step(kind, mode)
            return
        g = self.graphs.get((kind, mode))
        if g is None:
# ... 146 lines not shown
```

tweediemix_amd/unet.py:

```python
from __future__ import annotations

import ctypes as C
import json
import os
from dataclasses import dataclass

import torch

from . import lib as L
from . import ops
from .weights import fold_layernorm, interleave_geglu

BF16 = torch.bfloat16
F32 = torch.float32


@dataclass
class UNetConfig:
    in_channels: int = 4
    out_channels: int = 4
    block_out_channels: tuple = (320, 640, 1280)
    layers_per_block: int = 2
    transformer_layers: tuple = (0, 2, 10)
    head_dim: int = 64
    cross_dim: int = 2048
    pooled_dim: int = 1280
    addition_time_embed_dim: int = 256
    norm_groups: int = 32

    @property
    def time_embed_dim(self):
        return self.block_out_channels[0] * 4

    @property
    def add_in_dim(self):
        return self.pooled_dim + 6 * self.addition_time_embed_dim


    @classmethod
    def from_diffusers(cls, cfg: dict):
        ch = tuple(cfg["block_out_channels"])
        tl = cfg.get("transformer_layers_per_block", 1)
        tl = tuple(tl) if isinstance(tl, (list, tuple)) else (tl,) * len(ch)
        down = cfg.get("down_block_types", ["CrossAttnDownBlock2D"] * len(ch))
        tl = tuple(n if "CrossAttn" in t else 0 for n, t in zip(tl, down))
        heads = cfg.get("attention_head_dim", 8)
        heads = tuple(heads) if isinstance(heads, (list, tuple)) else (heads,) * len(ch)
        hd = {c // h for c, h, n in zip(ch, heads, tl) if n}
        if hd != {64}:
            raise ValueError(f"attention head size {sorted(hd)}: the attention kernel is built for 64 (SDXL)")
        add = cfg.get("addition_time_embed_dim", 256)
        return cls(in_channels=cfg.get("in_channels", 4), out_channels=cfg.get("out_channels", 4), block_out_channels=ch,
                   layers_per_block=cfg.get("layers_per_block", 2), transformer_layers=tl, head_dim=64,
                   cross_dim=cfg.get("cross_attention_dim", 2048),
                   pooled_dim=cfg.get("projection_class_embeddings_input_dim", 2816) - 6 * add,
                   addition_time_embed_dim=add, norm_groups=cfg.get("norm_num_groups", 32))


SDXL = UNetConfig()
TINY = UNetConfig(block_out_channels=(64, 128, 256), transformer_layers=(0, 1, 2), cross_dim=128,
                  pooled_dim=64, addition_time_embed_dim=32)


def transformer_sites(cfg: UNetConfig):
    out = []
    ch = cfg.block_out_channels
    nb = len(ch)
    for bi in range(nb):
        for j in range(cfg.layers_per_block):
            if cfg.transformer_layers[bi]:
                out.append((f"down_blocks.{bi}.attentions.{j}", ch[bi], cfg.transformer_layers[bi]))
    out.append(("mid_block.attentions.0", ch[-1], cfg.transformer_layers[-1]))
    for ui in range(nb):
        bi = nb - 1 - ui
        for j in range(cfg.layers_per_block + 1):
            if cfg.transformer_layers[bi]:
                out.append((f"up_blocks.{ui}.attentions.{j}", ch[bi], cfg.transformer_layers[bi]))
    return out


def attention_blocks(cfg: UNetConfig):
    return [(f"{p}.transformer_blocks.{i}", c) for p, c, n in transformer_sites(cfg) for i in range(n)]


class UNetWeights:

    def __init__(self, cfg: UNetConfig, sd: dict, device="cuda", concepts=None, lora_mode="merged"):
        self.cfg, self.device = cfg, torch.device(device)
        self.kind = concepts[0] if concepts else "none"
        self.K = len(concepts[1]) if concepts else 0
        assert lora_mode in ("merged", "lowrank")
        self.lora_mode = lora_mode if self.kind == "lora" else "merged"
        self._fp8 = {}
        self._tproj = None
        dev = self.device
        t = {}

        def g(name):
            return sd[name].to(dev)

        def bf(x):
            return x.to(dev, BF16).contiguous()

        def f32(x):
            return x.to(dev, F32).contiguous()

        for name, v in sd.items():
            if name.endswith(".bias") or ".norm" in name and name.endswith(".weight") or name.startswith("conv_norm_out"):
                t[name] = f32(v)
        t["conv_in.weight"] = f32(g("conv_in.weight").permute(0, 2, 3, 1))
        t["conv_out.weight"] = bf(g("conv_out.weight").permute(0, 2, 3, 1))
        for name, v in sd.items():
            if not name.endswith(".weight") or name in ("conv_in.weight", "conv_out.weight"):
                continue
            if v.dim() == 4 and v.shape[-1] == 3:
                t[name] = bf(v.to(dev).permute(0, 2, 3, 1))
            elif v.dim() == 4:
                t[name] = bf(v.to(dev).reshape(v.shape[0], v.shape[1]))
            elif v.dim() == 2 and ".attn" not in name and ".ff.net.0.proj" not in name:
                t[name] = bf(v)
        lora = concepts[1] if self.kind == "lora" else None
        custom = concepts[1] if self.kind == "custom" else None

        def merged(base, key, which):
            rows = [base.to(dev, F32)]
            for csd in lora:
                kd, ku = f"{key}.processor.to_{which}_lora.down.weight", f"{key}.processor.to_{which}_lora.up.weight"
                if kd in csd and ku in csd:
                    rows.append(rows[0] + csd[ku].to(dev, F32) @ csd[kd].to(dev, F32))
                else:
                    rows.append(rows[0])
            return torch.stack(rows)

        def lowrank(key, base, a, whiches, norm=None):
            nw, nsets = len(whiches), 1 + len(lora)
            P = 4 * nw
            assert nsets * P <= 64, "low-rank LoRA: (1 + concepts) x 4 x fused projections must fit the 64 pad columns"
            N, Kin = base.shape
            n1 = N // nw
            U = torch.zeros(N, 64, device=dev, dtype=F32)
            Dm = torch.zeros(nsets * P, Kin, device=dev, dtype=F32)
# ... 127 lines not shown
        lst = self.free.get(nbytes)
        if lst:
            buf = lst.pop()
        else:
            buf = torch.empty(nbytes, dtype=torch.uint8, device=self.device)
            self.bufs.append(buf)
            self.total += nbytes
        tns = buf.view(dtype)[:n].view(*shape)
        tns._arena_buf = buf
        return tns

    def put(self, *ts):
        for tns in ts:
            buf = tns._arena_buf
            self.free.setdefault(buf.numel(), []).append(buf)
            for cs, _c in getattr(tns, "_cs", None) or ():
                self.put(cs)
            tns._cs = None


_TUNE_CACHE = {}
SHARED = "shared|" 
ROUTED = "routed|"
_TUNE_FILE = os.environ.get("TMIX_TUNE_FILE", os.path.join(os.path.dirname(os.path.abspath(__file__)), "tuned_gfx950.json"))


def load_tune_table(path=None):
    path = _TUNE_FILE if path is None else path
    if path and os.path.exists(path):
        with open(path) as f:
            _TUNE_CACHE.update({k: int(v) for k, v in json.load(f).items()})
    return len(_TUNE_CACHE)


def save_tune_table(path):
    with open(path, "w") as f:
        json.dump(dict(sorted(_TUNE_CACHE.items())), f, indent=0)


def tune_lookup(ctx, key):
    c = _TUNE_CACHE.get(ctx + key)
    if c is None and ctx:
        c = _TUNE_CACHE.get(key)
        if ctx == SHARED and c in L.TILE_EXCLUSIVE:
            c = None
    return c


load_tune_table()


def hint_policy(B, h, w):
    small_call = B * h * w <= 4 * 128 * 128
    cap = int(float(os.environ.get("TMIX_PF_CAP_MB", "8" if small_call else "0")) * (1 << 20))
    over = int(float(os.environ.get("TMIX_PF_CAP_OVER_MB", "20")) * (1 << 20))
    return cap, over


def hint_bytes(nbytes, cap, over):
    return min(nbytes, cap) if cap and nbytes > over else nbytes


@dataclass
class TokenMapSpec:
    tokens: tuple
    row0: int = 1
    row_step: int = 2
    n_rows: int = 1
    levels: tuple | None = None


def attention_levels(cfg: UNetConfig):
    return tuple(bi for bi, n in enumerate(cfg.transformer_layers) if n)


class UNetPlan:

    token_spec = None
    token_maps = None
    _tok_arr = None

    def __init__(self, W: UNetWeights, B: int, h: int, w: int, kv: KVCache, pooled: torch.Tensor,
                 time_ids: torch.Tensor, routed: bool = False, autotune: bool = True, row_sets=None,
                 latent=None, eps=None, shared: bool = False, t_dev=None, fp8: bool = False, token_maps: TokenMapSpec | None = None):
        self._init_emit_state(W, B, h, w, hint_policy(B, h, w))
        self.fp8 = bool(fp8)
        self.fp8_chain_ff = not os.environ.get("TMIX_FP8_FF_ROWS")
        self.fp8_attn_out = not os.environ.get("TMIX_FP8_NO_ATTN_OUT")
        self.fp8_conv = not os.environ.get("TMIX_FP8_NO_CONV")
        self.fp8_conv_tile = int(os.environ.get("TMIX_FP8_CONV_TILE", "20"))
        self.fp8_tile = int(os.environ.get("TMIX_FP8_TILE", "21"))
        self.kv = kv
        self.row_sets = list(row_sets) if row_sets is not None else list(range(B))
        self.routed = bool(routed) and W.kind == "lora" and len(self.row_sets) == B and max(self.row_sets) <= W.K
        self.tune_ctx = SHARED if shared else (ROUTED if (self.routed and getattr(W, "lora_mode", "merged") != "lowrank") else "")
        self.lowrank = self.routed and getattr(W, "lora_mode", "merged") == "lowrank"
        if self.lowrank:
            assert not self.fp8, "low-rank LoRA runs the bf16 projections only"
            self.routed = False
            self._sets_dev = torch.tensor(self.row_sets, device=W.device, dtype=torch.int32)
        cfg = self.cfg
        assert kv.B == B
        dev = self.dev
        self.latent = latent if latent is not None else torch.zeros(B, cfg.in_channels, h, w, device=dev, dtype=F32)
        self.t_dev = t_dev if t_dev is not None else torch.zeros(B, device=dev, dtype=F32)
        self.eps = eps if eps is not None else torch.zeros(B, cfg.out_channels, h, w, device=dev, dtype=F32)
        assert self.latent.is_contiguous() and self.eps.is_contiguous() and self.latent.shape[0] == B
        tid = ops.timestep_embedding(time_ids.to(dev, F32).reshape(-1).contiguous(), cfg.addition_time_embed_dim)
        add_in = torch.cat([pooled.to(dev, F32), tid.reshape(B, -1)], dim=-1).contiguous()
        hid = ops.linear_small(add_in, W["add_embedding.linear_1.weight"], W["add_embedding.linear_1.bias"], act_out=True)
        self.aug = ops.linear_small(hid, W["add_embedding.linear_2.weight"], W["add_embedding.linear_2.bias"])
        torch.cuda.synchronize()
        self._gn_ws = ops.groupnorm_ws(B, 4096, cfg.norm_groups, dev)
        nb = len(cfg.block_out_channels)
        need = 1
        for pfx, cc, _n in transformer_sites(cfg):
            lvl = nb - 1 if pfx.startswith("mid") else int(pfx.split(".")[1]) if pfx.startswith("down") else nb - 1 - int(pfx.split(".")[1])
            need = max(need, ((cc + 127) // 128) * B * (h >> lvl) * (w >> lvl) * 2)
        self._ln_buf = torch.zeros(need, device=dev, dtype=F32)
        self._qattn = not os.environ.get("TMIX_NO_QATTN") and not self.fp8 and not self.lowrank and kv.Lk <= 80 and kv.ld == 80
        self.token_spec = token_maps
        self.token_maps = {}
        if token_maps is not None:
            tok = tuple(int(t) for t in token_maps.tokens)
            assert 1 <= len(tok) <= 8 and all(0 <= t < kv.Lk for t in tok), tok
            lv = attention_levels(self.cfg) if token_maps.levels is None else tuple(token_maps.levels)
            assert lv and all(l in attention_levels(self.cfg) for l in lv), lv
            self._tok_arr = ops.token_array(tok)
            for l in lv:
                self.token_maps[l] = torch.zeros(token_maps.n_rows, len(tok), (h >> l) * (w >> l), device=self.dev, dtype=F32)
        self._build()
        self._link_ln()
        if autotune:
            self.autotune()
        for m in self.token_maps.values():
            m.zero_()

    def _init_emit_state(self, W, B: int, h: int, w: int, hints):
        self.W, self.cfg, self.B, self.h, self.w = W, W.cfg, B, h, w
        self.lib = L.load()
        self.dev = W.device
        self.ops = []
        self.keep = []
        self.arena = _Arena(self.dev)
        self.flops = 0
        self.gemm_flops = 0
        self.launches = {"gemm": [], "conv": [], "attn": []}
        self.op_meta = {}
        self._tunable = []
        self._ln_links = []
        self._vt, self._rows_cache, self._attn_ws = {}, {}, {}
        self._pf_prev = None
        self._pf_on = not os.environ.get("TMIX_NO_PREFETCH")
        self._pf_cap, self._pf_cap_over = hints
        self._gn_fused = not os.environ.get("TMIX_GN_STATS_KERNEL")
        self._sc_fused = not os.environ.get("TMIX_SHORTCUT_GEMM")

    @staticmethod
    def _tune_key(kind, d):
        if kind == "gemm":
            return repr((kind, d.M, d.N, d.K, d.batch, d.epilogue, d.n_trans_begin >= 0, bool(d.residual), d.strideW != 0,
                         bool(d.row_stats_out), bool(d.ln_stats)))
        csc = d.S1_channels + d.S2_channels
        return repr((kind, d.B, d.H, d.W, d.Cin, d.Cout, d.mode) + ((csc,) if csc else ()))

    def autotune(self, reps=None):
        reps = reps or int(os.environ.get("TMIX_TUNE_REPS", "3"))
        tun = [(i, kind, d) for i, kind, d in self._tunable]
        force = int(os.environ.get("TMIX_FORCE_TILE", "0"))
        if force:
            for _i, _k, d in tun:
                d.tile_cfg = force
            self._link_ln()
            return
        keys = [self._tune_key(kind, d) for _i, kind, d in tun]
        ctx = self.tune_ctx
        lookup = lambda k: tune_lookup(ctx, k)
        if any(lookup(k) is None for k in keys):
            idx = {i: n for n, (i, _k, _d) in enumerate(tun)}
            st = torch.cuda.current_stream().cuda_stream
            best_t = {}
            cands = list(L.TILE_CANDIDATES)
            for _rep in range(reps):
                for cfg in cands:
                    for _i, kind, d in tun:
                        d.tile_cfg = cfg if kind == "gemm" else ops.conv_runs_as(d, cfg)
                    self._link_ln()
                    ev = [(torch.cuda.Event(enable_timing=True), torch.cuda.Event(enable_timing=True)) for _ in tun]
                    for i, (fn, args) in enumerate(self.ops):
                        n = idx.get(i)
                        if n is not None:
                            ev[n][0].record()
                        rc = fn(*args, st)
                        if rc:
                            L.check(rc, fn.__name__)
                        if n is not None:
                            ev[n][1].record()
                    torch.cuda.synchronize()
                    tot = {}
                    for n, k in enumerate(keys):
                        tot[k] = tot.get(k, 0.0) + ev[n][0].elapsed_time(ev[n][1])
                    for k, t in tot.items():
                        best_t[(k, cfg)] = min(best_t.get((k, cfg), float("inf")), t)
            first = {}
            for (_i, _kind, d), k in zip(tun, keys):
                first.setdefault(k, d)
            for k in set(keys):
                ok = [c for c in cands if k.startswith("('gemm'") or ops.conv_runs_as(first[k], c) == c]
                if k not in _TUNE_CACHE:
                    _TUNE_CACHE[k] = min(ok, key=lambda c: best_t[(k, c)])
                if SHARED + k not in _TUNE_CACHE:
                    _TUNE_CACHE[SHARED + k] = min([c for c in ok if c not in L.TILE_EXCLUSIVE], key=lambda c: best_t[(k, c)])
        for (_i, _kind, d), k in zip(tun, keys):
            d.tile_cfg = lookup(k)
        self._link_ln()
        torch.cuda.synchronize()

    def _emit(self, fn, *args):
        self.ops.append((fn, args))

    def _hint_weights(self, w):
        if not self._pf_on:
            return
        if self._pf_prev is not None:
            self._pf_prev[0], self._pf_prev[1] = w.data_ptr(), hint_bytes(w.numel() * w.element_size(), self._pf_cap, self._pf_cap_over)
        self._pf_prev = [None, 0]
        self.keep.append(w)
        self.ops.append((self.lib.tmix_gemm_prefetch_next, self._pf_prev))

    def _colstats(self, owner, rows, HW, Cc):
        if not self._gn_fused or HW % ops.COLSTATS_ROWS or HW > ops.COLSTATS_MAX_HW or rows % ops.COLSTATS_ROWS or Cc % 8:
            return None
        cs = self.arena.get(rows // ops.COLSTATS_ROWS, 2, Cc, dtype=F32)
        owner._cs = ((cs, Cc),)
        return cs

    def _gn_f8_ok(self, x, Cc, HW, x2=None):
        if not (self.fp8 and self.fp8_conv) or Cc % 128 or HW % 32:
            return False
        parts = getattr(x, "_cs", None)
        if x2 is not None:
            p2 = getattr(x2, "_cs", None)
            parts = (parts[0], p2[0]) if parts and p2 and len(parts) == 1 and len(p2) == 1 else None
        return bool(parts) and sum(c for _t, c in parts) == Cc

    def _gn(self, x, Cc, HW, name, eps, silu, out=None, x2=None, f8=False):
        if f8:
            out = (self.arena.get(self.B, HW, Cc, dtype=torch.uint8), self.arena.get(self.B * HW, Cc // 32, dtype=torch.uint8))
        else:
            out = out if out is not None else self.arena.get(self.B, HW, Cc)
        W = self.W
        C2 = 0 if x2 is None else x2.shape[-1]
        parts = getattr(x, "_cs", None)
        if x2 is not None:
            p2 = getattr(x2, "_cs", None)
            parts = (parts[0], p2[0]) if parts and p2 and len(parts) == 1 and len(p2) == 1 else None
        if parts and sum(c for _t, c in parts) == Cc and HW % ops.COLSTATS_ROWS == 0:
            (cs1, c1), (cs2, c2) = (parts[0], parts[1]) if len(parts) == 2 else (parts[0], (None, 0))
            if f8:
                self._emit(self.lib.tmix_groupnorm_nhwc_pre_f8, x.data_ptr(), Cc - C2, x2.data_ptr() if C2 else None, C2, out[0].data_ptr(), out[1].data_ptr(),
                           W[name + ".weight"].data_ptr(), W[name + ".bias"].data_ptr(), self._gn_ws.data_ptr(), self.B, HW, self.cfg.norm_groups, eps, int(silu),
                           cs1.data_ptr(), c1, cs2.data_ptr() if cs2 is not None else None, c2)
            else:
              self._emit(self.lib.tmix_groupnorm_nhwc_pre, x.data_ptr(), Cc - C2, x2.data_ptr() if C2 else None, C2, out.data_ptr(), W[name + ".weight"].data_ptr(),
                       W[name + ".bias"].data_ptr(), self._gn_ws.data_ptr(), self.B, HW, self.cfg.norm_groups, eps, int(silu),
                       cs1.data_ptr(), c1, cs2.data_ptr() if cs2 is not None else None, c2)
        else:
            assert not f8
            self._emit(self.lib.tmix_groupnorm_nhwc, x.data_ptr(), Cc - C2, x2.data_ptr() if C2 else None, C2, out.data_ptr(), W[name + ".weight"].data_ptr(),
                       W[name + ".bias"].data_ptr(), self._gn_ws.data_ptr(), self.B, HW, self.cfg.norm_groups, eps, int(silu))
        self.op_meta[len(self.ops) - 1] = ("norm", 0, ("norm", self.B, HW, Cc))
        return out

    def _gemm(self, a, w, out, fp8_key=None, f8_copy=None, a8=None, **kw):
        if fp8_key is not None and self.fp8:
            if a8 is not None:
                a = (a8.q.view(*a.shape), a8.scales)
            return self._gemm_fp8(a, fp8_key, out, f8_copy=f8_copy, **kw)
        if kw.get("row_stats_out") is not None:
            kw.setdefault("tile_cfg", 1)
        cs_owner = kw.pop("cs_owner", None)
        if cs_owner is not None and out.dim() == 2:
            kw["col_stats_out"] = self._colstats(cs_owner, out.shape[0], cs_owner.shape[1], out.shape[1])
        d = ops.make_gemm_desc(a, w, out, **kw)
        if f8_copy is not None:
            f8_copy.attach(d)
            self.keep.append(f8_copy)
        if kw.get("row_stats_out") is not None:
            self._ln_links.append((d, []))
        elif kw.get("ln_stats") is not None:
            self._ln_links[-1][1].append(d)
        self.keep.append(d)
        self._hint_weights(w)
        self._emit(self.lib.tmix_gemm_bf16, C.byref(d))
        fl = 2 * d.M * d.N * d.K * d.batch
        self.flops += fl
        self.gemm_flops += fl
        self.launches["gemm"].append((d, fl))
        self._tunable.append((len(self.ops) - 1, "gemm", d))
        self.op_meta[len(self.ops) - 1] = ("gemm", fl, d)
        return out

    def _gemm_fp8(self, a, key, out, f8_out=None, f8_copy=None, **kw):
        name, rows = key if isinstance(key, tuple) else (key, None)
        w8, sw = self.W.fp8(name, rows)
        flags = 0
        if isinstance(a, tuple):
            a8, sa = a
            flags |= L.F8_A_BLOCK_SCALES
            owned = ()
        else:
            K = a.shape[-1]
            a8 = self.arena.get(*a.shape, dtype=torch.uint8)
            sa = self.arena.get(*a.shape[:-1], dtype=torch.uint8)
            a2 = a.reshape(-1, K)
            assert a2.data_ptr() == a.data_ptr() and a2.stride(1) == 1
            self._emit(self.lib.tmix_quantize_fp8_rows, a2.data_ptr(), a2.stride(0), a8.data_ptr(), K, sa.data_ptr(), a2.shape[0], K)
            owned = (a8, sa)
        Ng, Kg = w8.shape[-2], w8.shape[-1]
        rows_g = a8.shape[-2] * (a8.shape[0] if a8.dim() == 3 else 1)
        lock = self.fp8_tile and f8_out is None and kw.get("out_t") is None and Kg % 128 == 0 and Ng % 160 == 0 and Ng <= 1280
        many = not (Kg >= 2560 or rows_g * Ng <= 4096 * 1280)
        if lock and (not many or kw.get("row_stats_out") is not None):
            kw.setdefault("tile_cfg", self.fp8_tile)
        if kw.get("row_stats_out") is not None:
            kw.setdefault("tile_cfg", 17)
        d = ops.make_gemm_desc(a8, w8, None if f8_out is not None else out, **kw)
        if f8_out is not None:
            c8, cs = f8_out
            assert kw.get("geglu") and c8.dim() == 2 and c8.stride(1) == 1 and cs.is_contiguous()
            d.C, d.ldc, d.strideC = c8.data_ptr(), c8.stride(0), 0
            d.Ct, d.ldct = cs.data_ptr(), cs.shape[1]
            flags |= L.F8_GEGLU_OUT
        d.reserved0 = flags
        if f8_copy is not None:
            f8_copy.attach(d)
            self.keep.append(f8_copy)
        if kw.get("row_stats_out") is not None:
            self._ln_links.append((d, []))
        elif kw.get("ln_stats") is not None:
            self._ln_links[-1][1].append(d)
        self.keep += [d, a8, sa]
        self._hint_weights(w8)
        self._emit(self.lib.tmix_gemm_fp8, C.byref(d), sa.data_ptr(), sw.data_ptr())
        fl = 2 * d.M * d.N * d.K * d.batch
        self.flops += fl
        self.gemm_flops += fl
# ... 254 lines not shown
                self._q_attn(h, a2 + ".q", self.kv.k[a2], self.kv.vt[a2], ao, S, Cc, st)
                self._proj(ao, a2 + ".out", h, S, Cc, bias=W[a2 + ".to_out.0.bias"], residual=h, stats_out=st, f8_copy=h8, a_full=ao)
                A.put(ao)
                q = None
            else:
                q = A.get(B, S, Cc)
                self._proj(h, a2 + ".q", q, S, Cc, ln=st, fp8=h8 is not None, a8=h8, a_full=h_full)
            if q is None:
                pass
            elif ao8 is not None:
                self._attn(q, self.kv.k[a2], self.kv.vt[a2], None, H, S, self.kv.Lk, f8_out=ao8)
                if lvl is not None:
                    self._token_maps(q, a2, H, S, lvl)
                A.put(q)
                self._proj(ao8.q.view(B, S, Cc), a2 + ".out", h, S, Cc, bias=W[a2 + ".to_out.0.bias"], residual=h, stats_out=st, f8_copy=h8, fp8=True, a8=ao8)
            else:
                ao_full = A.get(B, S, Cc + pad)
                ao = ao_full[:, :, :Cc] if pad else ao_full
                self._attn(q, self.kv.k[a2], self.kv.vt[a2], ao, H, S, self.kv.Lk)
                if lvl is not None:
                    self._token_maps(q, a2, H, S, lvl)
                A.put(q)
                self._proj(ao, a2 + ".out", h, S, Cc, bias=W[a2 + ".to_out.0.bias"], residual=h, stats_out=st, f8_copy=h8, a_full=ao_full)
                A.put(ao_full)
            if self.fp8 and self.fp8_chain_ff:
                f = A.get(B * S, 4 * Cc, dtype=torch.uint8)
                fs = A.get(4 * Cc // 32, B * S, dtype=torch.uint8)
                self._gemm_fp8((h8.q, h8.scales) if h8 is not None else h.view(B * S, Cc), tb + ".ff1", None, f8_out=(f, fs),
                               bias=W[tb + ".ff1.bias"], geglu=True, ln_stats=st, ln_colsum=W[tb + ".ff1.colsum"])
                self._gemm_fp8((f, fs), tb + ".ff.net.2.weight", h.view(B * S, Cc), bias=W[tb + ".ff.net.2.bias"],
                               residual=h.view(B * S, Cc), row_stats_out=st if i + 1 < n else None,
                               f8_copy=h8 if i + 1 < n else None)
                A.put(f, fs)
                continue
            f = A.get(B * S, 4 * Cc)
            self._gemm(h.view(B * S, Cc), W[tb + ".ff1"], f, bias=W[tb + ".ff1.bias"], geglu=True,
                       ln_stats=st, ln_colsum=W[tb + ".ff1.colsum"], fp8_key=tb + ".ff1")
            self._gemm(f, W[tb + ".ff.net.2.weight"], h.view(B * S, Cc), bias=W[tb + ".ff.net.2.bias"], residual=h.view(B * S, Cc),
                       row_stats_out=st if i + 1 < n else None, fp8_key=tb + ".ff.net.2.weight")
            A.put(f)
        out = A.get(B, S, Cc)
        self._gemm(h.view(B * S, Cc), W[name + ".proj_out.weight"], out.view(B * S, Cc), bias=W[name + ".proj_out.bias"],
                   residual=x.view(B * S, Cc), cs_owner=out)
        A.put(h_full)
        if h8 is not None:
            A.put(h8buf)
        if ao8buf is not None:
            A.put(ao8buf)
        return out

    def _cat(self, x1, C1, x2, C2, HW):
        out = self.arena.get(self.B, HW, C1 + C2)
        self._emit(self.lib.tmix_concat_channels, x1.data_ptr(), C1, x2.data_ptr(), C2, out.data_ptr(), self.B * HW)
        p1, p2 = getattr(x1, "_cs", None), getattr(x2, "_cs", None)
        if self._gn_fused and p1 and p2 and len(p1) == 1 and len(p2) == 1:
            out._cs = (p1[0], p2[0])
            x1._cs = x2._cs = None
        return out

    def _build(self):
        cfg, W, B, A = self.cfg, self.W, self.B, self.arena
        lib = self.lib
        ch = cfg.block_out_channels
        C0, T = ch[0], cfg.time_embed_dim
        nb = len(ch)
        tsin = torch.empty(B, C0, device=self.dev, dtype=F32)
        thid = torch.empty(B, T, device=self.dev, dtype=F32)
        emb = torch.empty(B, T, device=self.dev, dtype=F32)
        self.keep += [tsin, thid, emb]
        self._emit(lib.tmix_timestep_embedding, self.t_dev.data_ptr(), tsin.data_ptr(), B, C0)
        self._emit(lib.tmix_linear_small, tsin.data_ptr(), W["time_embedding.linear_1.weight"].data_ptr(),
                   W["time_embedding.linear_1.bias"].data_ptr(), None, thid.data_ptr(), B, T, C0, 0, 1)
        self._emit(lib.tmix_linear_small, thid.data_ptr(), W["time_embedding.linear_2.weight"].data_ptr(),
                   W["time_embedding.linear_2.bias"].data_ptr(), self.aug.data_ptr(), emb.data_ptr(), B, T, T, 0, 1)
        tw, tb_, starts, names = W.stacked_time_proj()
        tall = torch.empty(B * tw.shape[0], device=self.dev, dtype=F32)
        self.keep.append(tall)
        self._emit(lib.tmix_linear_small_sections, emb.data_ptr(), tw.data_ptr(), tb_.data_ptr(), tall.data_ptr(), B, tw.shape[0], T, 0,
                   starts.data_ptr(), len(names))
        hs = starts.tolist()
        self._temb = {n: tall[hs[i] * B:hs[i + 1] * B].view(B, hs[i + 1] - hs[i]) for i, n in enumerate(names)}
        Hh, Ww = self.h, self.w
        x = A.get(B, Hh * Ww, C0)
        self._emit(lib.tmix_conv_in, self.latent.data_ptr(), W["conv_in.weight"].data_ptr(), W["conv_in.bias"].data_ptr(),
                   x.data_ptr(), B, cfg.in_channels, Hh, Ww, C0)
        skips = [(x, C0)]
        ci = C0
        for bi, co in enumerate(ch):
            for j in range(cfg.layers_per_block):
                xin = x
                x = self._resnet(xin, ci, co, Hh, Ww, f"down_blocks.{bi}.resnets.{j}", emb)
                if cfg.transformer_layers[bi]:
                    x2 = self._t2d(x, co, Hh, Ww, f"down_blocks.{bi}.attentions.{j}", cfg.transformer_layers[bi])
                    A.put(x)
                    x = x2
                ci = co
                skips.append((x, co))
            if bi < nb - 1:
                x = self._conv(x, f"down_blocks.{bi}.downsamplers.0.conv", Hh, Ww, co, co, mode=L.CONV_S2)
                Hh, Ww = Hh // 2, Ww // 2
                skips.append((x, co))
        cm = ch[-1]
        x2 = self._resnet(x, cm, cm, Hh, Ww, "mid_block.resnets.0", emb)
        x3 = self._t2d(x2, cm, Hh, Ww, "mid_block.attentions.0", cfg.transformer_layers[-1])
        A.put(x2)
        x = self._resnet(x3, cm, cm, Hh, Ww, "mid_block.resnets.1", emb)
        A.put(x3)
        for ui, co in enumerate(reversed(ch)):
            bi = nb - 1 - ui
            for j in range(cfg.layers_per_block + 1):
                sk, cs = skips.pop()
                if self._sc_ok(ci + cs, co, ci, cs):
                    xn = self._resnet(x, ci + cs, co, Hh, Ww, f"up_blocks.{ui}.resnets.{j}", emb, x2=sk)
                    A.put(x, sk)
                    x = xn
                else:
                    xc = self._cat(x, ci, sk, cs, Hh * Ww)
                    A.put(x, sk)
                    x = self._resnet(xc, ci + cs, co, Hh, Ww, f"up_blocks.{ui}.resnets.{j}", emb)
                    A.put(xc)
                if cfg.transformer_layers[bi]:
                    x2 = self._t2d(x, co, Hh, Ww, f"up_blocks.{ui}.attentions.{j}", cfg.transformer_layers[bi])
                    A.put(x)
                    x = x2
                ci = co
            if ui < nb - 1:
                x2 = self._conv(x, f"up_blocks.{ui}.upsamplers.0.conv", Hh, Ww, co, co, mode=L.CONV_UP2)
                A.put(x)
                x = x2
                Hh, Ww = Hh * 2, Ww * 2
        y = self._gn(x, C0, Hh * Ww, "conv_norm_out", 1e-5, True)
        A.put(x)
        self._emit(lib.tmix_conv_out, y.data_ptr(), W["conv_out.weight"].data_ptr(), W["conv_out.bias"].data_ptr(),
                   self.eps.data_ptr(), B, C0, Hh, Ww, cfg.out_channels)
        self.flops += 2 * B * Hh * Ww * 9 * (cfg.in_channels * C0 + C0 * cfg.out_channels)
        self.ops = [(fn, tuple(a)) for fn, a in self.ops]

    def issued_meta(self):
        return [self.op_meta[i] for i in range(len(self.ops)) if i in self.op_meta]

    def run(self, stream=None):
        st = stream if stream is not None else torch.cuda.current_stream().cuda_stream
        for fn, args in self.ops:
            rc = fn(*args, st)
            if rc:
                L.check(rc, fn.__name__)

    def __call__(self, latent, t):
        self.latent.copy_(latent)
        self.t_dev.fill_(float(t))
        self.run()
        return self.eps

    def norm_condition(self, latent, t):
        self.latent.copy_(latent)
        self.t_dev.fill_(float(t))
        st = torch.cuda.current_stream().cuda_stream
        prods = {id(d) for d, _c in self._ln_links}
        out = []
        for i, (fn, args) in enumerate(self.ops):
            rc = fn(*args, st)
            if rc:
                L.check(rc, fn.__name__)
            m = self.op_meta.get(i)
            if not m or m[0] not in ("gemm", "gemm_fp8") or id(m[2]) not in prods:
                continue
            d = m[2]
            torch.cuda.synchronize()
            parts = ops.stats_parts(d.N, d.tile_cfg)
            base = (d.row_stats_out - self._ln_buf.data_ptr()) // 4
            rows = torch.arange(d.M, device=self.dev)
            s = torch.zeros(d.batch, d.M, 2, device=self.dev, dtype=torch.float64)
            for bz in range(d.batch):
                for q in range(parts):
                    off = base + bz * d.strideStatsOut + (q * d.ldStatsOut + rows) * 2
                    s[bz, :, 0] += self._ln_buf[off].double()
                    s[bz, :, 1] += self._ln_buf[off + 1].double()
            mean = s[..., 0] / d.N
            var = (s[..., 1] / d.N - mean * mean).clamp_min(1e-30)
            r = (mean.abs() / var.sqrt()).flatten()
            out.append((i, d.M * d.batch, d.N, r.max().item(), r.median().item()))
        torch.cuda.synchronize()
        return out


LN_COND_WARN = 16.0


def refine_group(self, top=14, reps=9, verbose=False, cands=None, only_kind=None):
    def timed():
        self.run()
        torch.cuda.synchronize()
        g = torch.cuda.CUDAGraph()
        with torch.cuda.graph(g):
            self.run()
        for _ in range(2):
            g.replay()
        import time as _time
        ts = []
        burst = 3
        for _ in range(reps):
            torch.cuda.synchronize()
            t0 = _time.perf_counter()
            for _b in range(burst):
                g.replay()
            torch.cuda.synchronize()
            ts.append(1e3 * (_time.perf_counter() - t0) / burst)
        return sorted(ts)[len(ts) // 2]

    plans = _plans_of(self)
    weight, members = {}, {}
    for p in plans:
        for _i, kind, d in p._tunable:
            k = p._tune_key(kind, d)
            fl = 2.0 * d.M * d.N * d.K * d.batch if kind == "gemm" else 2.0 * d.B * d.H * d.W * d.Cout * (9 * d.Cin + d.S1_channels + d.S2_channels)
            weight[k] = weight.get(k, 0.0) + fl
            members.setdefault(k, []).append((p, kind, d))
# ... 130 lines not shown
```

Measured before the change: 31.98.

## Fuse UNet edge ops: dedup conv_in rows, one-launch groupnorm, GN into conv_out

Adds a conv_in kernel that computes each shared latent only once and replicates it across the rows_per_latent batch rows, also emitting column statistics for the following groupnorm. Adds a single-launch groupnorm that reduces producer partials and applies the affine in one kernel for C >= 320. Fuses the final groupnorm+SiLU into an MFMA conv_out kernel so the normalized activation is never written out. These cut launches and memory traffic, at the cost of new kernels with strict eligibility conditions and the assumption that rows sharing a latent hold identical inputs.

After: 32.15, median of 6. About the same (+0.5%).

```diff
diff --git a/include/tmix.h b/include/tmix.h
--- a/include/tmix.h
+++ b/include/tmix.h
@@ -116,6 +116,8 @@
 
 int tmix_conv_in(const float* x_nchw, const float* w_ohwi, const float* bias, void* y_nhwc,
                  int B, int Cin, int H, int W, int Cout, void* stream);
+int tmix_conv_in_rows(const float* x_nchw, const float* w_ohwi, const float* bias, void* y_nhwc,
+                      int B, int Cin, int H, int W, int Cout, int rows_per_latent, float* col_stats_out, void* stream);
 int tmix_conv_in_pre(const float* x_nchw, const float* w_ohwi, const float* bias, void* y_nhwc,
                      int B, int Cin, int H, int W, int Cout, const float* pre_w, const float* pre_b, void* stream);
 int tmix_conv_out(const void* x_nhwc, const void* w_ohwi, const float* bias, float* y_nchw,
@@ -147,6 +149,14 @@
 int tmix_groupnorm_nhwc_pre_f8(const void* X1, int C1, const void* X2, int C2, void* Y8, void* scales, const float* gamma,
                                const float* beta, float* ws, int B, int64_t HW, int groups, float eps, int silu,
                                const float* cs1, int cs1_channels, const float* cs2, int cs2_channels, void* stream);
+int tmix_groupnorm_nhwc_pre1(const void* X1, int C1, const void* X2, int C2, void* Y, const float* gamma,
+                             const float* beta, float* ws, int B, int64_t HW, int groups, float eps, int silu,
+                             const float* cs1, int cs1_channels, const float* cs2, int cs2_channels, void* stream);
+int tmix_groupnorm_nhwc_pre_launches(int64_t HW, int C, int groups);
+int tmix_groupnorm_finalize_cs(const float* gamma, const float* beta, float* ws, int B, int64_t HW, int C, int groups, float eps,
+                               const float* cs1, int cs1_channels, const float* cs2, int cs2_channels, void* stream);
+int tmix_conv_out_gn(const void* x_nhwc, const float* scale_shift, int silu, const void* w_ohwi, const float* bias, float* y_nchw,
+                     int B, int Cin, int H, int W, int Cout, void* stream);
 int tmix_layernorm(const void* X, void* Y, const float* gamma, const float* beta, int64_t rows, int C,
                    float eps, void* stream);
 int tmix_zero(void* ptr, int64_t nbytes, void* stream);
diff --git a/tweediemix_amd/csrc/norm_misc.hip b/tweediemix_amd/csrc/norm_misc.hip
--- a/tweediemix_amd/csrc/norm_misc.hip
+++ b/tweediemix_amd/csrc/norm_misc.hip
@@ -167,6 +167,12 @@
     return x * __builtin_amdgcn_rcpf(1.0f + __builtin_amdgcn_exp2f(-1.4426950408889634f * x));
 }
 
+__device__ __forceinline__ float gn_affine(float x, float2 k, int silu) {
+    float y = x * k.x + k.y;
+    if (silu) y = silu_fast(y);
+    return y;
+}
+
 __device__ __forceinline__ float gn_quad_max(float x) {
     float y = __int_as_float(__builtin_amdgcn_update_dpp(0, __float_as_int(x), 0xB1, 0xf, 0xf, false));
     x = fmaxf(x, y);
@@ -210,12 +216,7 @@
             if (i + u * 256 < i1) {
                 float f[8]; unpack8(raw[u], f);
 #pragma unroll
-                for (int j = 0; j < 8; ++j) {
-                    const float2 k = s_ss[cc[u] + j];
-                    float y = f[j] * k.x + k.y;
-                    if (silu) y = silu_fast(y);
-                    f[j] = y;
-                }
+                for (int j = 0; j < 8; ++j) f[j] = gn_affine(f[j], s_ss[cc[u] + j], silu);
                 if constexpr (F8) {
                     const uint4 pk = pack8(f);
                     unpack8(pk, f);
@@ -336,6 +337,132 @@
         return gpw;
     }
     return 0;
+}
+
+#ifndef GN1_T
+#define GN1_T 1024
+#endif
+#ifndef GN1_MAXP
+#define GN1_MAXP 8
+#endif
+#ifndef GN1_ITEMS
+#define GN1_ITEMS 2560
+#endif
+constexpr int GN1_MAX_HW = 4096;
+static_assert(GN1_T >= 512 && GN1_T % 64 == 0, "the group combine uses 8 threads per group, up to 64 groups");
+__host__ __device__ inline int gn1_gpw(int64_t HW, int C, int groups) {
+    const int cpg = C / groups, want = HW > 1024 ? 64 : 120;
+    int fit = 0;
+    for (int gpw = 1; gpw <= groups; ++gpw) {
+        if (groups % gpw || ((gpw * cpg) & 7)) continue;
+        if (gpw * cpg > GN1_T) break;
+        fit = gpw;
+        if (gpw * cpg >= want) break;
+    }
+    return fit;
+}
+__host__ __device__ inline int gn1_ppc(int64_t HW, int sc) {
+    int64_t P = (HW * (sc >> 3) + GN1_ITEMS - 1) / GN1_ITEMS;
+    if (P > GN1_MAXP) P = GN1_MAXP;
+    if (P < 1) P = 1;
+    return (int)((HW + P - 1) / P);
+}
+static bool gn1_eligible(int64_t HW, int C, int groups) {
+    return HW > 0 && C > 0 && groups > 0 && groups <= 64 && !(C % groups) && !(C % 8) && !(HW % TMIX_COLSTATS_ROWS) && HW <= GN1_MAX_HW && gn1_gpw(HW, C, groups) > 0;
+}
+
+__global__ void __launch_bounds__(GN1_T) gn_pre1_kernel(const bf16_t* __restrict__ X1, int C1, const bf16_t* __restrict__ X2, int C2, bf16_t* __restrict__ Y,
+                                                        const float* __restrict__ cs1, int ca, const float* __restrict__ cs2, int cb,
+                                                        const float* __restrict__ gamma, const float* __restrict__ beta, int HW, int groups, int gpw, int ppc,
+                                                        float eps, int silu, unsigned long long* prof) {
+    __shared__ float r_s[GN1_T], r_q[GN1_T];
+    __shared__ double c_s[GN1_T], c_q[GN1_T];
+    __shared__ float g_ms[2 * 64];
+    __shared__ float2 s_ss[GN1_T];
+    const int tid = threadIdx.x;
+    const unsigned long long pt0 = (prof && tid == 0) ? prof_enter(prof, (blockIdx.x | blockIdx.y | blockIdx.z) == 0, 0) : 0;
+    const int C = C1 + C2, cpg = C / groups, sc = gpw * cpg, nv = sc >> 3;
+    const int b = blockIdx.z, c0 = blockIdx.y * sc;
+    const int nblk = HW / TMIX_COLSTATS_ROWS;
+    float gm = 0.f, bt = 0.f;
+    if (tid < sc) { gm = gamma[c0 + tid]; bt = beta[c0 + tid]; }
+    {
+        const int J = GN1_T / sc, j = tid / sc, c = tid - j * sc;
+        if (j < J) {
+            const int cg = c0 + c;
+            const float* row; int Cs;
+            if (cg < ca) { row = cs1 + (int64_t)b * nblk * 2 * ca + cg; Cs = ca; }
+            else         { row = cs2 + (int64_t)b * nblk * 2 * cb + (cg - ca); Cs = cb; }
+            row += (int64_t)j * 2 * Cs;
+            const int64_t step = (int64_t)J * 2 * Cs;
+            float s = 0.f, q = 0.f;
+            int blk = j;
+            for (; blk + 3 * J < nblk; blk += 4 * J, row += 4 * step) {
+                const float a0 = row[0], b0 = row[Cs], a1 = row[step], b1 = row[step + Cs];
+                const float a2 = row[2 * step], b2 = row[2 * step + Cs], a3 = row[3 * step], b3 = row[3 * step + Cs];
+                s += (a0 + a1) + (a2 + a3); q += (b0 + b1) + (b2 + b3);
+            }
+            for (; blk < nblk; blk += J, row += step) { s += row[0]; q += row[Cs]; }
+            r_s[tid] = s; r_q[tid] = q;
+        }
+        __syncthreads();
+        if (tid < sc) {
+            double a = 0.0, d = 0.0;
+            for (int k = 0; k < J; ++k) { a += (double)r_s[k * sc + tid]; d += (double)r_q[k * sc + tid]; }
+            c_s[tid] = a; c_q[tid] = d;
+        }
+    }
+    __syncthreads();
+    if (tid < gpw * 8) {
+        const int g = tid >> 3, l = tid & 7;
+        double a = 0.0, d = 0.0;
+        for (int k = l; k < cpg; k += 8) { a += c_s[g * cpg + k]; d += c_q[g * cpg + k]; }
+#pragma unroll
+        for (int o = 4; o > 0; o >>= 1) { a += __shfl_xor(a, o); d += __shfl_xor(d, o); }
+        if (l == 0) {
+            const double n = (double)HW * cpg, mean = a / n;
+            double var = d / n - mean * mean; if (var < 0.0) var = 0.0;
+            g_ms[2 * g] = (float)mean; g_ms[2 * g + 1] = (float)(1.0 / sqrt(var + (double)eps));
+        }
+    }
+    __syncthreads();
+    if (tid < sc) {
+        const int g = tid / cpg;
+        const float k = g_ms[2 * g + 1] * gm;
+        s_ss[tid] = make_float2(k, bt - g_ms[2 * g] * k);
+    }
+    __syncthreads();
+    const int rs = GN1_T / nv, v = tid % nv, slot = tid / nv;
+    if (slot < rs) {
+        float2 k[8];
+#pragma unroll
+        for (int j = 0; j < 8; ++j) k[j] = s_ss[v * 8 + j];
+        const int cg = c0 + v * 8;
+        const bf16_t* src; int ld;
+        if (cg < C1) { src = X1 + (int64_t)b * HW * C1 + cg; ld = C1; } else { src = X2 + (int64_t)b * HW * C2 + (cg - C1); ld = C2; }
+        bf16_t* dst = Y + (int64_t)b * HW * C + cg;
+        const int p0 = blockIdx.x * ppc, p1 = min(HW, p0 + ppc);
+        int row = p0 + slot;
+        for (; row + rs < p1; row += 2 * rs) {
+            uint4 raw[2];
+#pragma unroll
+            for (int u = 0; u < 2; ++u) raw[u] = *(const uint4*)(src + (int64_t)(row + u * rs) * ld);
+#pragma unroll
+            for (int u = 0; u < 2; ++u) {
+                float f[8]; unpack8(raw[u], f);
+#pragma unroll
+                for (int j = 0; j < 8; ++j) f[j] = gn_affine(f[j], k[j], silu);
+                *(uint4*)(dst + (int64_t)(row + u * rs) * C) = pack8(f);
+            }
+        }
+        for (; row < p1; row += rs) {
+            float f[8]; unpack8(*(const uint4*)(src + (int64_t)row * ld), f);
+#pragma unroll
+            for (int j = 0; j < 8; ++j) f[j] = gn_affine(f[j], k[j], silu);
+            *(uint4*)(dst + (int64_t)row * C) = pack8(f);
+        }
+    }
+    if (prof && tid == 0) prof_leave(prof, 0, pt0, pt0, pt0);
 }
 
 __global__ void __launch_bounds__(256) layernorm_kernel(const bf16_t* __restrict__ X, bf16_t* __restrict__ Y,
@@ -565,6 +692,82 @@
         }
         if (live) *(uint4*)(y + pix * Cout + c0) = pack8(o);
     }
+    }
+}
+
+template <int CIN>
+__global__ void __launch_bounds__(256) conv_in_rows_kernel(const float* __restrict__ x, const float* __restrict__ w, const float* __restrict__ bias,
+                                                           bf16_t* __restrict__ y, float* __restrict__ cs, int B, int H, int W, int Cout, int r) {
+    extern __shared__ __attribute__((aligned(16))) float s_w[];
+    constexpr int KK = 9 * CIN;
+    const int tid = threadIdx.x, lane = tid & 63;
+    const int q = __builtin_amdgcn_readfirstlane(tid >> 6);
+    bf16_t* s_y = (bf16_t*)(s_w + Cout * KK);
+    const int ldy = Cout + 8, nv = Cout >> 3;
+    for (int i = tid; i < Cout * KK / 4; i += 256) ((float4*)s_w)[i] = ((const float4*)w)[i];
+    __syncthreads();
+    const int HW = H * W;
+    const int64_t npix = (int64_t)(B / r) * HW;
+    for (int64_t tile = blockIdx.x; tile * 64 < npix; tile += gridDim.x) {
+    int64_t pix = tile * 64 + lane;
+    if (pix > npix - 1) pix = npix - 1;
+    const int s = (int)(pix / HW); const int rem = (int)(pix - (int64_t)s * HW);
+    const int b = s * r;
+    const int oy = rem / W, ox = rem - oy * W;
+    float patch[KK];
+#pragma unroll
+    for (int ky = 0; ky < 3; ++ky)
+#pragma unroll
+        for (int kx = 0; kx < 3; ++kx) {
+            const int iy = oy + ky - 1, ix = ox + kx - 1;
+            const bool ok = iy >= 0 && iy < H && ix >= 0 && ix < W;
+#pragma unroll
+            for (int ci = 0; ci < CIN; ++ci) patch[(ky * 3 + kx) * CIN + ci] = ok ? x[(((int64_t)b * CIN + ci) * H + iy) * W + ix] : 0.f;
+        }
+    const int cpq = Cout / 4;
+    for (int c0 = q * cpq; c0 < (q + 1) * cpq; c0 += 8) {
+        float o[8];
+#pragma unroll 2
+        for (int j = 0; j < 8; ++j) {
+            const float* wr = s_w + (c0 + j) * KK;
+            float a = bias ? bias[c0 + j] : 0.f;
+#pragma unroll
+            for (int k = 0; k < KK; ++k) a += patch[k] * wr[k];
+            o[j] = a;
+        }
+        *(uint4*)(s_y + lane * ldy + c0) = pack8(o);
+    }
+    __syncthreads();
+    const int nlive = (int)min((int64_t)64, npix - tile * 64);
+    for (int idx = tid; idx < nlive * nv; idx += 256) {
+        const int p = idx / nv, v = idx - p * nv;
+        const uint4 pk = *(const uint4*)(s_y + p * ldy + v * 8);
+        const int64_t gp = tile * 64 + p;
+        const int ss = (int)(gp / HW);
+        bf16_t* dst = y + (((int64_t)ss * r) * HW + (gp - (int64_t)ss * HW)) * Cout + v * 8;
+        for (int i = 0; i < r; ++i) *(uint4*)(dst + (int64_t)i * HW * Cout) = pk;
+    }
+    if (cs) {
+        const int nd = Cout >> 1;
+        for (int idx = tid; idx < 2 * nd; idx += 256) {
+            const int h = idx / nd, d = idx - h * nd;
+            if (h * 32 >= nlive) continue;
+            float s0 = 0.f, s1 = 0.f, q0 = 0.f, q1 = 0.f;
+            for (int p = h * 32; p < h * 32 + 32; ++p) {
+                const uint32_t u = *(const uint32_t*)(s_y + p * ldy + 2 * d);
+                const float f0 = bf2f((bf16_t)(u & 0xffff)), f1 = bf2f((bf16_t)(u >> 16));
+                s0 += f0; s1 += f1; q0 += f0 * f0; q1 += f1 * f1;
+            }
+            const int64_t gp = tile * 64 + h * 32;
+            const int ss = (int)(gp / HW);
+            float* o2 = cs + ((((int64_t)ss * r) * (HW / 32) + (gp - (int64_t)ss * HW) / 32) * 2) * Cout + 2 * d;
+            for (int i = 0; i < r; ++i) {
+                *(float2*)(o2 + (int64_t)i * (HW / 32) * 2 * Cout) = make_float2(s0, s1);
+                *(float2*)(o2 + (int64_t)i * (HW / 32) * 2 * Cout + Cout) = make_float2(q0, q1);
+            }
+        }
+    }
+    __syncthreads();
     }
 }
 
@@ -607,6 +810,84 @@
     }
 }
 
+constexpr int COG_TH = 4, COG_TW = 32, COG_PW = COG_TW + 2, COG_PIX = (COG_TH + 2) * COG_PW, COG_T = 512;
+__global__ void __launch_bounds__(COG_T) conv_out_gn_kernel(const bf16_t* __restrict__ x, const float2* __restrict__ ss, int silu, const bf16_t* __restrict__ w,
+                                                          const float* __restrict__ bias, float* __restrict__ y, int B, int H, int W, int Cin, int Cout,
+                                                          unsigned long long* prof) {
+    extern __shared__ __attribute__((aligned(16))) bf16_t s_p[];
+    const int ldp = Cin + 8, nv = Cin >> 3;
+    float2* s_ss = (float2*)(s_p + COG_PIX * ldp);
+    const int tid = threadIdx.x, lane = tid & 63, wv = tid >> 6;
+    const int tw = (W + COG_TW - 1) / COG_TW, th = (H + COG_TH - 1) / COG_TH;
+    int t = blockIdx.x;
+    const int b = t / (th * tw); t -= b * th * tw;
+    const int ty = t / tw, tx = t - ty * tw;
+    const int y0 = ty * COG_TH - 1, x0 = tx * COG_TW - 1;
+    for (int c = tid; c < Cin; c += COG_T) s_ss[c] = ss[(int64_t)b * Cin + c];
+    __syncthreads();
+    constexpr int U = 8;
+    for (int i0 = tid; i0 < COG_PIX * nv; i0 += COG_T * U) {
+        uint4 raw[U]; bool in[U];
+#pragma unroll
+        for (int u = 0; u < U; ++u) {
+            const int idx = i0 + u * COG_T;
+            const int pp = idx / nv, v = idx - pp * nv;
+            const int pr = pp / COG_PW, pc = pp - pr * COG_PW;
+            const int iy = y0 + pr, ix = x0 + pc;
+            in[u] = idx < COG_PIX * nv && iy >= 0 && iy < H && ix >= 0 && ix < W;
+            if (in[u]) raw[u] = *(const uint4*)(x + (((int64_t)b * H + iy) * W + ix) * Cin + v * 8);
+        }
+#pragma unroll
+        for (int u = 0; u < U; ++u) {
+            const int idx = i0 + u * COG_T;
+            if (idx >= COG_PIX * nv) break;
+            const int pp = idx / nv, v = idx - pp * nv;
+            uint4 o = make_uint4(0, 0, 0, 0);
+            if (in[u]) {
+                float f[8]; unpack8(raw[u], f);
+#pragma unroll
+                for (int j = 0; j < 8; ++j) f[j] = gn_affine(f[j], s_ss[v * 8 + j], silu);
+                o = pack8(f);
+            }
+            *(uint4*)(s_p + pp * ldp + v * 8) = o;
+        }
+    }
+    __syncthreads();
+    const int fr = lane & 15, fg = lane >> 4, trow = wv & 3, half = wv >> 2;
+    const int co = fr < Cout ? fr : Cout - 1;
+    const bf16_t* wrow = w + (int64_t)co * 9 * Cin + fg * 8;
+    f32x4 acc = {0.f, 0.f, 0.f, 0.f};
+    const int nkc = Cin >> 5, nk = 9 * nkc;
+    constexpr int WQ = 8;
+    frag_ab wq[WQ];
+#pragma unroll
+    for (int u = 0; u < WQ; ++u) if (u < nk) wq[u] = *(const frag_ab*)(wrow + u * 32);
+    const bf16_t* abase = s_p + (trow * COG_PW + half * 16 + fr) * ldp + fg * 8;
+    for (int k0 = 0; k0 < nk; k0 += WQ) {
+#pragma unroll
+        for (int u = 0; u < WQ; ++u) {
+            const int k = k0 + u;
+            if (k < nk) {
+                const int tap = k / nkc, c = (k - tap * nkc) << 5;
+                const int ky = tap / 3, kx = tap - ky * 3;
+                acc = __builtin_amdgcn_mfma_f32_16x16x32_bf16(*(const frag_ab*)(abase + (ky * COG_PW + kx) * ldp + c), wq[u], acc, 0, 0, 0);
+                if (k + WQ < nk) wq[u] = *(const frag_ab*)(wrow + (k + WQ) * 32);
+            }
+        }
+    }
+    const int oy = ty * COG_TH + trow;
+    if (fr < Cout && oy < H) {
+        const float bv = bias ? bias[fr] : 0.f;
+        float* dst = y + (((int64_t)b * Cout + fr) * H + oy) * W;
+#pragma unroll
+        for (int r = 0; r < 4; ++r) {
+            const int ox = tx * COG_TW + half * 16 + fg * 4 + r;
+            if (ox < W) dst[ox] = acc[r] + bv;
+        }
+    }
+    if (prof && tid == 0) prof_leave(prof, 0, 0, 0, 0);
+}
+
 }
 
 extern "C" int tmix_groupnorm_ws_chunks(int64_t HW) { return gn_chunks(HW); }
@@ -681,6 +962,73 @@
                                           const float* cs1, int cs1_channels, const float* cs2, int cs2_channels, void* stream) {
     if (!scales) TMIX_FAIL(TMIX_EINVAL, "groupnorm_pre_f8: null scale array");
     return gn_pre_entry(X1, C1, X2, C2, Y8, scales, gamma, beta, ws, B, HW, groups, eps, silu, cs1, cs1_channels, cs2, cs2_channels, stream);
+}
+
+extern "C" int tmix_groupnorm_nhwc_pre_launches(int64_t HW, int C, int groups) {
+    if (HW <= 0 || C <= 0 || groups <= 0 || (C % groups)) return 0;
+    return gn1_eligible(HW, C, groups) ? 1 : 2;
+}
+
+extern "C" int tmix_groupnorm_nhwc_pre1(const void* X1, int C1, const void* X2, int C2, void* Y, const float* gamma,
+                                        const float* beta, float* ws, int B, int64_t HW, int groups, float eps, int silu,
+                                        const float* cs1, int cs1_channels, const float* cs2, int cs2_channels, void* stream) {
+    if (!X1 || !Y || !gamma || !beta || !ws || !cs1) TMIX_FAIL(TMIX_EINVAL, "groupnorm_pre1: null pointer");
+    if (C2 > 0 && !X2) TMIX_FAIL(TMIX_EINVAL, "groupnorm_pre1: C2 > 0 but X2 is null");
+    const int C = C1 + C2;
+    if (cs1_channels <= 0 || cs2_channels < 0 || cs1_channels + cs2_channels != C || (cs2_channels > 0 && !cs2))
+        TMIX_FAIL(TMIX_EINVAL, "groupnorm_pre1: the partials cover %d + %d channels, the tensor has %d", cs1_channels, cs2_channels, C);
+    if (B <= 0 || B > 65535 || HW <= 0 || C <= 0) TMIX_FAIL(TMIX_ESHAPE, "groupnorm_pre1: empty problem");
+    if (C1 < 0 || C2 < 0 || (C1 % 8) || (C2 % 8) || C > GN_MAX_C || groups <= 0 || groups > 64 || (C % groups) || C / groups > 256) TMIX_FAIL(TMIX_ESHAPE, "groupnorm_pre1: C1=%d C2=%d groups=%d unsupported", C1, C2, groups);
+    if (!gn1_eligible(HW, C, groups))
+        TMIX_FAIL(TMIX_ESHAPE, "groupnorm_pre1: HW=%lld must be a multiple of %d and <= %d, with a slab of whole groups of <= %d channels (C=%d groups=%d): use tmix_groupnorm_nhwc_pre",
+                  (long long)HW, TMIX_COLSTATS_ROWS, GN1_MAX_HW, GN1_T, C, groups);
+    if (!aligned16(X1) || (X2 && !aligned16(X2)) || !aligned16(Y)) TMIX_FAIL(TMIX_EALIGN, "groupnorm_pre1: pointers must be 16-byte aligned");
+    const int gpw = gn1_gpw(HW, C, groups), sc = gpw * (C / groups), ppc = gn1_ppc(HW, sc);
+    unsigned long long* prof = tmix_prof_take();
+    gn_pre1_kernel<<<dim3((unsigned)((HW + ppc - 1) / ppc), groups / gpw, B), GN1_T, 0, (hipStream_t)stream>>>(
+        (const bf16_t*)X1, C1, (const bf16_t*)X2, C2, (bf16_t*)Y, cs1, cs1_channels, cs2, cs2_channels, gamma, beta, (int)HW, groups, gpw, ppc, eps, silu, prof);
+    TMIX_LAUNCH_CHECK();
+    return TMIX_OK;
+}
+
+static thread_local unsigned long long* t_gn_open_slot = nullptr;
+
+extern "C" int tmix_groupnorm_finalize_cs(const float* gamma, const float* beta, float* ws, int B, int64_t HW, int C, int groups, float eps,
+                                          const float* cs1, int cs1_channels, const float* cs2, int cs2_channels, void* stream) {
+    if (!gamma || !beta || !ws || !cs1) TMIX_FAIL(TMIX_EINVAL, "groupnorm_finalize_cs: null pointer");
+    if (cs1_channels <= 0 || cs2_channels < 0 || cs1_channels + cs2_channels != C || (cs2_channels > 0 && !cs2))
+        TMIX_FAIL(TMIX_EINVAL, "groupnorm_finalize_cs: the partials cover %d + %d channels, the tensor has %d", cs1_channels, cs2_channels, C);
+    if (B <= 0 || B > 65535 || HW <= 0 || C <= 0) TMIX_FAIL(TMIX_ESHAPE, "groupnorm_finalize_cs: empty problem");
+    if ((C % 8) || C > GN_MAX_C || groups <= 0 || groups > 64 || (C % groups) || C / groups > 256) TMIX_FAIL(TMIX_ESHAPE, "groupnorm_finalize_cs: C=%d groups=%d unsupported", C, groups);
+    if (HW % TMIX_COLSTATS_ROWS) TMIX_FAIL(TMIX_ESHAPE, "groupnorm_finalize_cs: HW=%lld must be a multiple of %d", (long long)HW, TMIX_COLSTATS_ROWS);
+    t_gn_open_slot = tmix_prof_take();
+    float2* ss = (float2*)(ws + (int64_t)B * GN_T * groups * 2);
+    gn_finalize_cs_kernel<<<dim3(groups, B), GN_CS_T, 0, (hipStream_t)stream>>>(cs1, cs1_channels, cs2, cs2_channels, gamma, beta, ss, HW, groups, eps, t_gn_open_slot);
+    TMIX_LAUNCH_CHECK();
+    return TMIX_OK;
+}
+
+extern "C" int tmix_conv_out_gn(const void* x_nhwc, const float* scale_shift, int silu, const void* w_ohwi, const float* bias, float* y_nchw,
+                                int B, int Cin, int H, int W, int Cout, void* stream) {
+    unsigned long long* prof = t_gn_open_slot;
+    t_gn_open_slot = nullptr;
+    if (!x_nhwc || !scale_shift || !w_ohwi || !y_nchw) TMIX_FAIL(TMIX_EINVAL, "conv_out_gn: null pointer");
+    if (B <= 0 || H <= 0 || W <= 0 || Cin <= 0 || Cout <= 0 || Cout > 16 || (Cin % 32)) TMIX_FAIL(TMIX_ESHAPE, "conv_out_gn: Cin=%d (%%32) Cout=%d (<=16)", Cin, Cout);
+    if (!aligned16(x_nhwc) || !aligned16(w_ohwi) || (((uintptr_t)scale_shift) & 7u)) TMIX_FAIL(TMIX_EALIGN, "conv_out_gn: x / w must be 16-byte aligned, scale_shift 8-byte");
+    const int smem = COG_PIX * (Cin + 8) * 2 + Cin * 8;
+    if (smem > 150 * 1024) TMIX_FAIL(TMIX_ESHAPE, "conv_out_gn: Cin=%d too deep for the LDS patch (%d bytes)", Cin, smem);
+    const int64_t nt = (int64_t)B * ((H + COG_TH - 1) / COG_TH) * ((W + COG_TW - 1) / COG_TW);
+    if (nt > 0x7fffffff) TMIX_FAIL(TMIX_ESHAPE, "conv_out_gn: too many tiles");
+    static int attr_smem = 0;
+    if (smem > 64 * 1024 && smem > attr_smem) {
+        hipError_t e = hipFuncSetAttribute((const void*)conv_out_gn_kernel, hipFuncAttributeMaxDynamicSharedMemorySize, smem);
+        if (e != hipSuccess) TMIX_FAIL((int)e, "hipFuncSetAttribute: %s", hipGetErrorString(e));
+        attr_smem = smem;
+    }
+    conv_out_gn_kernel<<<(unsigned)nt, COG_T, smem, (hipStream_t)stream>>>((const bf16_t*)x_nhwc, (const float2*)scale_shift, silu, (const bf16_t*)w_ohwi, bias, y_nchw,
+                                                                          B, H, W, Cin, Cout, prof);
+    TMIX_LAUNCH_CHECK();
+    return TMIX_OK;
 }
 
 extern "C" int tmix_layernorm(const void* X, void* Y, const float* gamma, const float* beta, int64_t rows, int C,
@@ -1047,6 +1395,42 @@
     return TMIX_OK;
 }
 
+extern "C" int tmix_conv_in_rows(const float* x_nchw, const float* w_ohwi, const float* bias, void* y_nhwc,
+                                 int B, int Cin, int H, int W, int Cout, int rows_per_latent, float* col_stats_out, void* stream) {
+    if (!x_nchw || !w_ohwi || !y_nhwc) TMIX_FAIL(TMIX_EINVAL, "conv_in_rows: null pointer");
+    if (B <= 0 || H <= 0 || W <= 0 || Cout <= 0) TMIX_FAIL(TMIX_ESHAPE, "conv_in_rows: bad shape");
+    if (rows_per_latent < 1 || (B % rows_per_latent)) TMIX_FAIL(TMIX_ESHAPE, "conv_in_rows: rows_per_latent=%d must divide B=%d", rows_per_latent, B);
+    if (Cout % 32) TMIX_FAIL(TMIX_ESHAPE, "conv_in_rows: Cout=%d must be a multiple of 32", Cout);
+    if (Cin != 3 && Cin != 4 && Cin != 8) TMIX_FAIL(TMIX_ESHAPE, "conv_in_rows: Cin=%d (3, 4 or 8)", Cin);
+    if ((Cout * 9 * Cin) % 4) TMIX_FAIL(TMIX_ESHAPE, "conv_in_rows: Cout*9*Cin must be a multiple of 4");
+    if ((int64_t)H * W > (1 << 30)) TMIX_FAIL(TMIX_ESHAPE, "conv_in_rows: image too large");
+    if (col_stats_out && (((int64_t)H * W) % TMIX_COLSTATS_ROWS))
+        TMIX_FAIL(TMIX_ESHAPE, "conv_in_rows: H*W=%lld must be a multiple of %d for the column partials (32-row blocks must not straddle images)", (long long)H * W, TMIX_COLSTATS_ROWS);
+    if (!aligned16(y_nhwc) || !aligned16(w_ohwi) || (col_stats_out && !aligned16(col_stats_out))) TMIX_FAIL(TMIX_EALIGN, "conv_in_rows: output, weights and partials must be 16-byte aligned");
+    const int smem = Cout * 9 * Cin * 4 + 64 * (Cout + 8) * 2;
+    if (smem > 150 * 1024) TMIX_FAIL(TMIX_ESHAPE, "conv_in_rows: Cout=%d too large for the LDS weight stage", Cout);
+    const int64_t npix = (int64_t)(B / rows_per_latent) * H * W;
+    const int64_t ntiles = (npix + 63) / 64;
+    const int per_cu = smem > 80 * 1024 ? 1 : (smem > 52 * 1024 ? 2 : 3);
+    const unsigned nb = (unsigned)(ntiles < 256 * per_cu ? ntiles : 256 * per_cu);
+    static int attr_smem[3] = {0, 0, 0};
+    const int slot = Cin == 8 ? 2 : (Cin == 4 ? 1 : 0);
+    if (smem > 64 * 1024 && smem > attr_smem[slot]) {
+        hipError_t e = Cin == 8 ? hipFuncSetAttribute((const void*)conv_in_rows_kernel<8>, hipFuncAttributeMaxDynamicSharedMemorySize, smem)
+                     : Cin == 4 ? hipFuncSetAttribute((const void*)conv_in_rows_kernel<4>, hipFuncAttributeMaxDynamicSharedMemorySize, smem)
+                                : hipFuncSetAttribute((const void*)conv_in_rows_kernel<3>, hipFuncAttributeMaxDynamicSharedMemorySize, smem);
+        if (e != hipSuccess) TMIX_FAIL((int)e, "hipFuncSetAttribute: %s", hipGetErrorString(e));
+        attr_smem[slot] = smem;
+    }
+    hipStream_t st = (hipStream_t)stream;
+    bf16_t* y = (bf16_t*)y_nhwc;
+    if (Cin == 8) conv_in_rows_kernel<8><<<nb, 256, smem, st>>>(x_nchw, w_ohwi, bias, y, col_stats_out, B, H, W, Cout, rows_per_latent);
+    else if (Cin == 3) conv_in_rows_kernel<3><<<nb, 256, smem, st>>>(x_nchw, w_ohwi, bias, y, col_stats_out, B, H, W, Cout, rows_per_latent);
+    else          conv_in_rows_kernel<4><<<nb, 256, smem, st>>>(x_nchw, w_ohwi, bias, y, col_stats_out, B, H, W, Cout, rows_per_latent);
+    TMIX_LAUNCH_CHECK();
+    return TMIX_OK;
+}
+
 extern "C" int tmix_conv_out(const void* x_nhwc, const void* w_ohwi, const float* bias, float* y_nchw,
                              int B, int Cin, int H, int W, int Cout, void* stream) {
     if (!x_nhwc || !w_ohwi || !y_nchw) TMIX_FAIL(TMIX_EINVAL, "conv_out: null pointer");
diff --git a/tweediemix_amd/lib.py b/tweediemix_amd/lib.py
--- a/tweediemix_amd/lib.py
+++ b/tweediemix_amd/lib.py
@@ -65,6 +65,7 @@
     "tmix_conv3x3_nhwc": (C.c_int, [C.POINTER(ConvDesc), vp]),
     "tmix_conv3x3_nhwc_fp8": (C.c_int, [C.POINTER(ConvDesc), vp, vp, vp]),
     "tmix_conv_in": (C.c_int, [vp, vp, vp, vp, C.c_int, C.c_int, C.c_int, C.c_int, C.c_int, vp]),
+    "tmix_conv_in_rows": (C.c_int, [vp, vp, vp, vp, C.c_int, C.c_int, C.c_int, C.c_int, C.c_int, C.c_int, vp, vp]),
     "tmix_conv_in_pre": (C.c_int, [vp, vp, vp, vp, C.c_int, C.c_int, C.c_int, C.c_int, C.c_int, vp, vp, vp]),
     "tmix_softmax_rows": (C.c_int, [vp, i64, vp, i64, i64, C.c_int, f32, vp]),
     "tmix_softmax_rows_causal": (C.c_int, [vp, i64, vp, i64, i64, C.c_int, f32, C.c_int, vp]),
@@ -87,6 +88,11 @@
                                       C.c_int, vp]),
     "tmix_groupnorm_nhwc_pre": (C.c_int, [vp, C.c_int, vp, C.c_int, vp, vp, vp, vp, C.c_int, i64, C.c_int, f32,
                                           C.c_int, vp, C.c_int, vp, C.c_int, vp]),
+    "tmix_groupnorm_nhwc_pre1": (C.c_int, [vp, C.c_int, vp, C.c_int, vp, vp, vp, vp, C.c_int, i64, C.c_int, f32,
+                                           C.c_int, vp, C.c_int, vp, C.c_int, vp]),
+    "tmix_groupnorm_nhwc_pre_launches": (C.c_int, [i64, C.c_int, C.c_int]),
+    "tmix_groupnorm_finalize_cs": (C.c_int, [vp, vp, vp, C.c_int, i64, C.c_int, C.c_int, f32, vp, C.c_int, vp, C.c_int, vp]),
+    "tmix_conv_out_gn": (C.c_int, [vp, vp, C.c_int, vp, vp, vp, C.c_int, C.c_int, C.c_int, C.c_int, C.c_int, vp]),
     "tmix_groupnorm_nhwc_pre_f8": (C.c_int, [vp, C.c_int, vp, C.c_int, vp, vp, vp, vp, vp, C.c_int, i64, C.c_int, f32,
                                              C.c_int, vp, C.c_int, vp, C.c_int, vp]),
     "tmix_layernorm": (C.c_int, [vp, vp, vp, vp, i64, C.c_int, f32, vp]),
diff --git a/tweediemix_amd/ops.py b/tweediemix_amd/ops.py
--- a/tweediemix_amd/ops.py
+++ b/tweediemix_amd/ops.py
@@ -338,6 +338,21 @@
     return out
 
 
+def conv_in_rows(x_nchw, w_ohwi, bias, rows_per_latent=1, out=None, col_stats_out=None):
+    _need_cuda(x_nchw, w_ohwi)
+    lib = L.load()
+    B, Cin, H, W = x_nchw.shape
+    Cout = w_ohwi.shape[0]
+    assert x_nchw.dtype == torch.float32 and w_ohwi.dtype == torch.float32 and x_nchw.is_contiguous() and w_ohwi.is_contiguous()
+    if out is None:
+        out = torch.empty(B, H, W, Cout, device=x_nchw.device, dtype=BF16)
+    if col_stats_out is not None:
+        assert col_stats_out.dtype == torch.float32 and col_stats_out.is_contiguous() and col_stats_out.numel() >= (B * H * W // COLSTATS_ROWS) * 2 * Cout
+    L.check(lib.tmix_conv_in_rows(_p(x_nchw), _p(w_ohwi), _p(bias), _p(out), B, Cin, H, W, Cout, int(rows_per_latent), _p(col_stats_out), _stream()),
+            "tmix_conv_in_rows")
+    return out
+
+
 def conv_out(x_nhwc, w_ohwi, bias, out=None):
     _need_cuda(x_nhwc, w_ohwi)
     lib = L.load()
@@ -347,6 +362,30 @@
     if out is None:
         out = torch.empty(B, Cout, H, W, device=x_nhwc.device, dtype=torch.float32)
     L.check(lib.tmix_conv_out(_p(x_nhwc), _p(w_ohwi), _p(bias), _p(out), B, Cin, H, W, Cout, _stream()), "tmix_conv_out")
+    return out
+
+
+def groupnorm_scale_shift(ws, B, C, groups=32):
+    n = L.load().tmix_groupnorm_ws_floats(B, C, groups)
+    return ws[n - 2 * B * C:n].view(B, C, 2)
+
+
+def conv_out_gn(x_nhwc, gamma, beta, colstats, w_ohwi, bias, groups=32, eps=1e-5, silu=True, out=None, ws=None):
+    _need_cuda(x_nhwc, w_ohwi, gamma, beta)
+    lib = L.load()
+    B, H, W, Cin = x_nhwc.shape
+    Cout = w_ohwi.shape[0]
+    assert x_nhwc.dtype == BF16 and w_ohwi.dtype == BF16 and x_nhwc.is_contiguous() and w_ohwi.is_contiguous() and gamma.dtype == torch.float32
+    cs1, cs2 = colstats
+    ca, cb = cs1.shape[-1], (0 if cs2 is None else cs2.shape[-1])
+    if ws is None:
+        ws = groupnorm_ws(B, Cin, groups, x_nhwc.device)
+    if out is None:
+        out = torch.empty(B, Cout, H, W, device=x_nhwc.device, dtype=torch.float32)
+    L.check(lib.tmix_groupnorm_finalize_cs(_p(gamma), _p(beta), _p(ws), B, H * W, Cin, groups, float(eps), _p(cs1), ca, _p(cs2), cb, _stream()),
+            "tmix_groupnorm_finalize_cs")
+    L.check(lib.tmix_conv_out_gn(_p(x_nhwc), groupnorm_scale_shift(ws, B, Cin, groups).data_ptr(), int(bool(silu)), _p(w_ohwi), _p(bias), _p(out),
+                                 B, Cin, H, W, Cout, _stream()), "tmix_conv_out_gn")
     return out
 
 
@@ -402,12 +441,13 @@
     return torch.empty(L.load().tmix_groupnorm_ws_floats(B, C, groups), device=device, dtype=torch.float32)
 
 
-def groupnorm(x1, gamma, beta, groups=32, eps=1e-5, silu=False, x2=None, out=None, ws=None, colstats=None, f8_out=None):
+def groupnorm(x1, gamma, beta, groups=32, eps=1e-5, silu=False, x2=None, out=None, ws=None, colstats=None, f8_out=None, one_launch=False):
     _need_cuda(x1, gamma, beta)
     lib = L.load()
     B, HW, C1 = x1.shape[0], x1.numel() // (x1.shape[0] * x1.shape[-1]), x1.shape[-1]
     C2 = 0 if x2 is None else x2.shape[-1]
     assert x1.is_contiguous() and (x2 is None or x2.is_contiguous()) and gamma.dtype == torch.float32
+    assert not one_launch or (colstats is not None and f8_out is None), "the one-launch form reads producer partials and writes bf16"
     assert f8_out is None or colstats is not None, "the e4m3 output exists for the producer-statistics form (tmix_groupnorm_nhwc_pre_f8)"
     if out is None and f8_out is None:
         out = torch.empty(*x1.shape[:-1], C1 + C2, device=x1.device, dtype=BF16)
@@ -426,12 +466,17 @@
             L.check(lib.tmix_groupnorm_nhwc_pre_f8(_p(x1), C1, _p(x2), C2, _p(y8), _p(s8), _p(gamma), _p(beta), _p(ws), B, HW, groups,
                                                    float(eps), int(bool(silu)), _p(cs1), ca, _p(cs2), cb, _stream()), "tmix_groupnorm_nhwc_pre_f8")
             return f8_out
-        L.check(lib.tmix_groupnorm_nhwc_pre(_p(x1), C1, _p(x2), C2, _p(out), _p(gamma), _p(beta), _p(ws), B, HW, groups,
-                                            float(eps), int(bool(silu)), _p(cs1), ca, _p(cs2), cb, _stream()), "tmix_groupnorm_nhwc_pre")
+        fn = lib.tmix_groupnorm_nhwc_pre1 if one_launch else lib.tmix_groupnorm_nhwc_pre
+        L.check(fn(_p(x1), C1, _p(x2), C2, _p(out), _p(gamma), _p(beta), _p(ws), B, HW, groups,
+                   float(eps), int(bool(silu)), _p(cs1), ca, _p(cs2), cb, _stream()), fn.__name__)
         return out
     L.check(lib.tmix_groupnorm_nhwc(_p(x1), C1, _p(x2), C2, _p(out), _p(gamma), _p(beta), _p(ws), B, HW, groups,
                                     float(eps), int(bool(silu)), _stream()), "tmix_groupnorm_nhwc")
     return out
+
+
+def groupnorm_pre_launches(HW, C, groups=32):
+    return L.load().tmix_groupnorm_nhwc_pre_launches(HW, C, groups)
 
 
 def layernorm(x, gamma, beta, eps=1e-5, out=None):
diff --git a/tweediemix_amd/sampler.py b/tweediemix_amd/sampler.py
--- a/tweediemix_amd/sampler.py
+++ b/tweediemix_amd/sampler.py
@@ -126,13 +126,13 @@
             am = self.attention_masks
             spec = TokenMapSpec(tuple(am["flat"]), row0=1, row_step=2, n_rows=S, levels=am["levels"])
             return UNetPlan(self.W, B, self.h, self.w, KVCache(self.W, ehs, wsel), pooled, self.add_time_ids.repeat(B, 1),
-                            fp8=self.fp8, token_maps=spec)
+                            fp8=self.fp8, token_maps=spec, rows_per_latent=B // S)
         if self.n_streams > 1 and B % self.n_streams == 0 and B // self.n_streams >= self.min_rows_per_stream:
             return PlanGroup(self.W, self.h, self.w, ehs, wsel, pooled, self.add_time_ids.repeat(B, 1), routed,
                              self.n_streams, fp8=self.fp8)
         kv = KVCache(self.W, ehs, wsel)
         return UNetPlan(self.W, B, self.h, self.w, kv, pooled, self.add_time_ids.repeat(B, 1), routed=routed,
-                        row_sets=wsel if routed else None, fp8=self.fp8)
+                        row_sets=wsel if routed else None, fp8=self.fp8, rows_per_latent=B // S)
 
     def plan(self, kind):
         if kind not in self.plans:
diff --git a/tweediemix_amd/unet.py b/tweediemix_amd/unet.py
--- a/tweediemix_amd/unet.py
+++ b/tweediemix_amd/unet.py
@@ -57,6 +57,7 @@
                    addition_time_embed_dim=add, norm_groups=cfg.get("norm_num_groups", 32))
 
 
+GN_PRE1_MIN_C = 320
 SDXL = UNetConfig()
 TINY = UNetConfig(block_out_channels=(64, 128, 256), transformer_layers=(0, 1, 2), cross_dim=128,
                   pooled_dim=64, addition_time_embed_dim=32)
@@ -350,7 +351,10 @@
 
     def __init__(self, W: UNetWeights, B: int, h: int, w: int, kv: KVCache, pooled: torch.Tensor,
                  time_ids: torch.Tensor, routed: bool = False, autotune: bool = True, row_sets=None,
-                 latent=None, eps=None, shared: bool = False, t_dev=None, fp8: bool = False, token_maps: TokenMapSpec | None = None):
+                 latent=None, eps=None, shared: bool = False, t_dev=None, fp8: bool = False, token_maps: TokenMapSpec | None = None,
+                 rows_per_latent: int = 1):
+        assert rows_per_latent >= 1 and B % rows_per_latent == 0
+        self.rows_per_latent = int(rows_per_latent)
         self._init_emit_state(W, B, h, w, hint_policy(B, h, w))
         self.fp8 = bool(fp8)
         self.fp8_chain_ff = not os.environ.get("TMIX_FP8_FF_ROWS")
@@ -422,6 +426,8 @@
         self._pf_on = not os.environ.get("TMIX_NO_PREFETCH")
         self._pf_cap, self._pf_cap_over = hints
         self._gn_fused = not os.environ.get("TMIX_GN_STATS_KERNEL")
+        self._gn_pre1 = os.environ.get("TMIX_GN_PRE1", "1") != "0"
+        self._edge_fused = os.environ.get("TMIX_EDGE_FUSED", "1") != "0"
         self._sc_fused = not os.environ.get("TMIX_SHORTCUT_GEMM")
 
     @staticmethod
@@ -530,7 +536,8 @@
                            W[name + ".weight"].data_ptr(), W[name + ".bias"].data_ptr(), self._gn_ws.data_ptr(), self.B, HW, self.cfg.norm_groups, eps, int(silu),
                            cs1.data_ptr(), c1, cs2.data_ptr() if cs2 is not None else None, c2)
             else:
-              self._emit(self.lib.tmix_groupnorm_nhwc_pre, x.data_ptr(), Cc - C2, x2.data_ptr() if C2 else None, C2, out.data_ptr(), W[name + ".weight"].data_ptr(),
+              one = self._gn_pre1 and Cc >= GN_PRE1_MIN_C and self.lib.tmix_groupnorm_nhwc_pre_launches(HW, Cc, self.cfg.norm_groups) == 1
+              self._emit(self.lib.tmix_groupnorm_nhwc_pre1 if one else self.lib.tmix_groupnorm_nhwc_pre, x.data_ptr(), Cc - C2, x2.data_ptr() if C2 else None, C2, out.data_ptr(), W[name + ".weight"].data_ptr(),
                        W[name + ".bias"].data_ptr(), self._gn_ws.data_ptr(), self.B, HW, self.cfg.norm_groups, eps, int(silu),
                        cs1.data_ptr(), c1, cs2.data_ptr() if cs2 is not None else None, c2)
         else:
@@ -951,8 +958,13 @@
         self._temb = {n: tall[hs[i] * B:hs[i + 1] * B].view(B, hs[i + 1] - hs[i]) for i, n in enumerate(names)}
         Hh, Ww = self.h, self.w
         x = A.get(B, Hh * Ww, C0)
-        self._emit(lib.tmix_conv_in, self.latent.data_ptr(), W["conv_in.weight"].data_ptr(), W["conv_in.bias"].data_ptr(),
-                   x.data_ptr(), B, cfg.in_channels, Hh, Ww, C0)
+        if self._edge_fused:
+            cs = self._colstats(x, B * Hh * Ww, Hh * Ww, C0)
+            self._emit(lib.tmix_conv_in_rows, self.latent.data_ptr(), W["conv_in.weight"].data_ptr(), W["conv_in.bias"].data_ptr(),
+                       x.data_ptr(), B, cfg.in_channels, Hh, Ww, C0, self.rows_per_latent, cs.data_ptr() if cs is not None else None)
+        else:
+            self._emit(lib.tmix_conv_in, self.latent.data_ptr(), W["conv_in.weight"].data_ptr(), W["conv_in.bias"].data_ptr(),
+                       x.data_ptr(), B, cfg.in_channels, Hh, Ww, C0)
         skips = [(x, C0)]
         ci = C0
         for bi, co in enumerate(ch):
@@ -998,10 +1010,19 @@
                 A.put(x)
                 x = x2
                 Hh, Ww = Hh * 2, Ww * 2
-        y = self._gn(x, C0, Hh * Ww, "conv_norm_out", 1e-5, True)
-        A.put(x)
-        self._emit(lib.tmix_conv_out, y.data_ptr(), W["conv_out.weight"].data_ptr(), W["conv_out.bias"].data_ptr(),
-                   self.eps.data_ptr(), B, C0, Hh, Ww, cfg.out_channels)
+        parts = getattr(x, "_cs", None)
+        if self._edge_fused and parts and len(parts) == 1 and parts[0][1] == C0 and (Hh * Ww) % ops.COLSTATS_ROWS == 0 and C0 % 32 == 0 and C0 <= 480 and cfg.out_channels <= 16:
+            self._emit(lib.tmix_groupnorm_finalize_cs, W["conv_norm_out.weight"].data_ptr(), W["conv_norm_out.bias"].data_ptr(), self._gn_ws.data_ptr(), B, Hh * Ww, C0,
+                       cfg.norm_groups, 1e-5, parts[0][0].data_ptr(), C0, None, 0)
+            self.op_meta[len(self.ops) - 1] = ("norm", 0, ("norm", B, Hh * Ww, C0))
+            self._emit(lib.tmix_conv_out_gn, x.data_ptr(), ops.groupnorm_scale_shift(self._gn_ws, B, C0, cfg.norm_groups).data_ptr(), 1, W["conv_out.weight"].data_ptr(),
+                       W["conv_out.bias"].data_ptr(), self.eps.data_ptr(), B, C0, Hh, Ww, cfg.out_channels)
+            A.put(x)
+        else:
+            y = self._gn(x, C0, Hh * Ww, "conv_norm_out", 1e-5, True)
+            A.put(x)
+            self._emit(lib.tmix_conv_out, y.data_ptr(), W["conv_out.weight"].data_ptr(), W["conv_out.bias"].data_ptr(),
+                       self.eps.data_ptr(), B, C0, Hh, Ww, cfg.out_channels)
         self.flops += 2 * B * Hh * Ww * 9 * (cfg.in_channels * C0 + C0 * cfg.out_channels)
         self.ops = [(fn, tuple(a)) for fn, a in self.ops]
 
```
